# yu45020/Text_Segmentation_Image_Inpainting

Hardware: NVIDIA H100
Metric: PartialConv UNet 512x512 images/sec (fwd+bwd) (higher is better)
Workload: dtype bf16

## Files before the change

text_segmentation_image_inpainting_b200/csrc/conv_k2r.cu:

```cuda
#include <string.h>

#include <algorithm>

#include "pcb_common.cuh"

namespace {

constexpr int K2R_N = 32;
constexpr int K2R_CO = 3;
constexpr int K2R_TAPS = 9;

size_t rup256(size_t v) { return (v + 255) / 256 * 256; }
size_t zbytes(const pcb_conv *c) { return rup256(static_cast<size_t>(c->n) * (c->h >> 1) * (c->w >> 1) * K2R_N * sizeof(bf16)); }

}

K2rPlan pcb_k2r_plan(const pcb_conv *c) {
    K2rPlan K;
    memset(&K, 0, sizeof(K));
    if (!pcb_smallco_eligible(c)) return K;
    if (c->kh != 3 || c->kw != 3 || c->pad_h != 1 || c->pad_w != 1 || c->cout > K2R_CO || c->nparts != 2) return K;
    if (c->ho != c->h || c->wo != c->w || ((c->h | c->w) & 1)) return K;
    K.pu = c->parts[0].x_up ? 0 : 1;
    K.ps = 1 - K.pu;
    const pcb_part &u = c->parts[K.pu], &v = c->parts[K.ps];
    if (!u.x_up || v.x_up || u.c < 32 || (u.c & 7) || v.c > 4) return K;
    if ((u.mask && u.mask_up != 1) || (v.mask && v.mask_up != 0)) return K;
    K.cu = u.c; K.cs = v.c;
    K.choff_u = K.pu == 0 ? 0 : c->parts[0].c;
    K.choff_s = K.ps == 0 ? 0 : c->parts[0].c;
    pcb_conv &S = K.sub;
    S.n = c->n; S.h = c->h >> 1; S.w = c->w >> 1; S.cin = u.c; S.cout = K2R_N; S.kh = S.kw = 1; S.stride = 1; S.pad_h = S.pad_w = 0; S.dil = 1;
    S.groups = 1; S.ho = S.h; S.wo = S.w; S.dtype = PCB_BF16; S.nparts = 1;
    S.parts[0] = u; S.parts[0].x_up = 0; S.parts[0].mask_up = 0;
    if (!pcb_tc_eligible(&S)) return K;
    pcb_tc_weight_layout(&S, &K.sub_fe, &K.sub_de);
    K.sub_fe = (K.sub_fe + 63) / 64 * 64;
    K.sub_de = (K.sub_de + 63) / 64 * 64;
    K.fwd_extra = K.sub_fe + 2 * static_cast<size_t>(K2R_N) * K.cu;
    K.dg_extra = K.sub_de;
    K.workspace = zbytes(c) + rup256(sizeof(float) * K2R_N * K.cu) + pcb_tc_workspace(&S);
    K.ok = true;
    return K;
}

namespace {

__global__ void k2r_weight_kernel(const float *__restrict__ w, float *__restrict__ wsub, int cout, int cin, int choff_u, int cu) {
    const int i = blockIdx.x * blockDim.x + threadIdx.x;
    if (i >= K2R_N * cu) return;
    const int k = i / cu, ch = i - k * cu;
    const int tap = k / K2R_CO, co = k - tap * K2R_CO;
    wsub[i] = (tap < K2R_TAPS && co < cout) ? w[(static_cast<long long>(co) * K2R_TAPS + tap) * cin + choff_u + ch] : 0.f;
}

__global__ void k2r_dw_scatter_kernel(const float *__restrict__ dwsub, float *__restrict__ dw, int cout, int cin, int choff_u, int cu) {
    const int i = blockIdx.x * blockDim.x + threadIdx.x;
    if (i >= K2R_TAPS * K2R_CO * cu) return;
    const int k = i / cu, ch = i - k * cu;
    const int tap = k / K2R_CO, co = k - tap * K2R_CO;
    if (co < cout) dw[(static_cast<long long>(co) * K2R_TAPS + tap) * cin + choff_u + ch] += dwsub[i];
}

struct K2rParams {
    int n, h, w, hs, ws, cout, cin, no_guard;
    const bf16 *z;
    const bf16 *v; int v_cstride;
    const uint8_t *mv;
    const bf16 *w_fwd; long long kf; int ktap, koff_s;
    const float *bias, *msum;
    bf16 *y; int y_cstride;
    const bf16 *dc; int dc_cstride;
    bf16 *d;
    float *dw; int choff_s;
};

__device__ __forceinline__ void bf4_to_float(const uint2 r, float (&f)[4]) {
    const __nv_bfloat162 *h = reinterpret_cast<const __nv_bfloat162 *>(&r);
    const float2 a = __bfloat1622float2(h[0]), b = __bfloat1622float2(h[1]);
    f[0] = a.x; f[1] = a.y; f[2] = b.x; f[3] = b.y;
}

template <int CS>
__global__ void __launch_bounds__(256) k2r_combine_kernel(const K2rParams P) {
    __shared__ float4 s_w[K2R_TAPS * K2R_CO];
    for (int i = threadIdx.x; i < K2R_TAPS * K2R_CO; i += blockDim.x) {
        const int tap = i / K2R_CO, co = i - tap * K2R_CO;
        float wv[4] = {0.f, 0.f, 0.f, 0.f};
        if (co < P.cout)
            for (int ch = 0; ch < CS; ++ch) wv[ch] = __bfloat162float(P.w_fwd[static_cast<long long>(co) * P.kf + static_cast<long long>(tap) * P.ktap + P.koff_s + ch]);
        s_w[i] = make_float4(wv[0], wv[1], wv[2], wv[3]);
    }
    __syncthreads();
    const long long total = static_cast<long long>(P.n) * P.hs * P.ws;
    for (long long idx = blockIdx.x * static_cast<long long>(blockDim.x) + threadIdx.x; idx < total; idx += static_cast<long long>(gridDim.x) * blockDim.x) {
        const int sx = static_cast<int>(idx % P.ws);
        const long long t = idx / P.ws;
        const int sy = static_cast<int>(t % P.hs), img = static_cast<int>(t / P.hs);
        float acc[4][K2R_CO];
#pragma unroll
        for (int ch = 0; ch < 4; ++ch)
#pragma unroll
            for (int co = 0; co < K2R_CO; ++co) acc[ch][co] = 0.f;
#pragma unroll
        for (int dy = -1; dy <= 1; ++dy) {
            const int yy = sy + dy;
            if (yy < 0 || yy >= P.hs) continue;
#pragma unroll
            for (int dx = -1; dx <= 1; ++dx) {
                const int xx = sx + dx;
                if (xx < 0 || xx >= P.ws) continue;
                const uint4 *row = reinterpret_cast<const uint4 *>(P.z + ((static_cast<long long>(img) * P.hs + yy) * P.ws + xx) * K2R_N);
                float zf[K2R_N];
#pragma unroll
                for (int q = 0; q < 4; ++q) {
                    const uint4 r = __ldg(row + q);
                    const __nv_bfloat162 *h = reinterpret_cast<const __nv_bfloat162 *>(&r);
#pragma unroll
                    for (int e = 0; e < 4; ++e) {
                        const float2 f = __bfloat1622float2(h[e]);
                        zf[q * 8 + 2 * e] = f.x; zf[q * 8 + 2 * e + 1] = f.y;
                    }
                }
#pragma unroll
                for (int a = 0; a < 2; ++a)
#pragma unroll
                    for (int b = 0; b < 2; ++b)
#pragma unroll
                        for (int tr = 0; tr < 3; ++tr)
#pragma unroll
                            for (int tc = 0; tc < 3; ++tc) {
                                const int ny = (a + tr + 1) / 2 - 1, nx = (b + tc + 1) / 2 - 1;
                                if (ny == dy && nx == dx) {
#pragma unroll
                                    for (int co = 0; co < K2R_CO; ++co) acc[a * 2 + b][co] += zf[(tr * 3 + tc) * K2R_CO + co];
                                }
                            }
            }
        }
        float xv[4][4][CS];
#pragma unroll
        for (int i = 0; i < 4; ++i) {
            const int y = 2 * sy - 1 + i;
#pragma unroll
            for (int j = 0; j < 4; ++j) {
                const int x = 2 * sx - 1 + j;
                bool ok = y >= 0 && y < P.h && x >= 0 && x < P.w;
                const long long q = (static_cast<long long>(img) * P.h + (ok ? y : 0)) * P.w + (ok ? x : 0);
                if (ok && P.mv) ok = P.mv[q] != 0;
                float f[4] = {0.f, 0.f, 0.f, 0.f};
                if (ok) bf4_to_float(__ldg(reinterpret_cast<const uint2 *>(P.v + q * P.v_cstride)), f);
#pragma unroll
                for (int ch = 0; ch < CS; ++ch) xv[i][j][ch] = f[ch];
            }
        }
#pragma unroll
        for (int tr = 0; tr < 3; ++tr)
#pragma unroll
            for (int tc = 0; tc < 3; ++tc)
#pragma unroll
                for (int co = 0; co < K2R_CO; ++co) {
                    const float4 wv = s_w[(tr * 3 + tc) * K2R_CO + co];
                    const float wq[4] = {wv.x, wv.y, wv.z, wv.w};
#pragma unroll
                    for (int a = 0; a < 2; ++a)
#pragma unroll
                        for (int b = 0; b < 2; ++b)
#pragma unroll
                            for (int ch = 0; ch < CS; ++ch) acc[a * 2 + b][co] = fmaf(wq[ch], xv[a + tr][b + tc][ch], acc[a * 2 + b][co]);
                }
#pragma unroll
        for (int a = 0; a < 2; ++a)
#pragma unroll
            for (int b = 0; b < 2; ++b) {
                const long long q = (static_cast<long long>(img) * P.h + 2 * sy + a) * P.w + 2 * sx + b;
                const float s = P.msum ? P.msum[q] : 1.f;
                const bool hole = (s == 0.f) && !P.no_guard;
                const float inv = hole ? 0.f : 1.0f / s;
                float o[8] = {0.f, 0.f, 0.f, 0.f, 0.f, 0.f, 0.f, 0.f};
#pragma unroll
                for (int co = 0; co < K2R_CO; ++co)
                    if (co < P.cout && !hole) o[co] = acc[a * 2 + b][co] * inv + (P.bias ? P.bias[co] : 0.f);
                Vec8<bf16>::store(P.y + q * P.y_cstride, o);
            }
    }
}

template <bool WG, int CS>
__global__ void __launch_bounds__(256) k2r_dbuild_kernel(const K2rParams P) {
    __shared__ float s_dw[WG ? K2R_TAPS * K2R_CO * 4 : 1];
    if (WG) {
        for (int i = threadIdx.x; i < K2R_TAPS * K2R_CO * 4; i += blockDim.x) s_dw[i] = 0.f;
        __syncthreads();
    }
    float gw[WG ? K2R_TAPS * K2R_CO : 1][WG ? CS : 1];
    if (WG) {
#pragma unroll
        for (int k = 0; k < K2R_TAPS * K2R_CO; ++k)
#pragma unroll
            for (int ch = 0; ch < CS; ++ch) gw[k][ch] = 0.f;
    }
    const long long total = static_cast<long long>(P.n) * P.hs * P.ws;
    for (long long idx = blockIdx.x * static_cast<long long>(blockDim.x) + threadIdx.x; idx < total; idx += static_cast<long long>(gridDim.x) * blockDim.x) {
        const int sx = static_cast<int>(idx % P.ws);
        const long long t = idx / P.ws;
        const int sy = static_cast<int>(t % P.hs), img = static_cast<int>(t / P.hs);
        float win[4][4][K2R_CO];
#pragma unroll
        for (int i = 0; i < 4; ++i) {
            const int y = 2 * sy - 1 + i;
#pragma unroll
            for (int j = 0; j < 4; ++j) {
                const int x = 2 * sx - 1 + j;
                const bool ok = y >= 0 && y < P.h && x >= 0 && x < P.w;
                float f[4] = {0.f, 0.f, 0.f, 0.f};
                if (ok) bf4_to_float(__ldg(reinterpret_cast<const uint2 *>(P.dc + ((static_cast<long long>(img) * P.h + y) * P.w + x) * P.dc_cstride)), f);
#pragma unroll
                for (int co = 0; co < K2R_CO; ++co) win[i][j][co] = f[co];
            }
        }
        if (P.d) {
            float dv[K2R_N];
#pragma unroll
            for (int k = K2R_TAPS * K2R_CO; k < K2R_N; ++k) dv[k] = 0.f;
#pragma unroll
            for (int tr = 0; tr < 3; ++tr)
#pragma unroll
                for (int tc = 0; tc < 3; ++tc)
#pragma unroll
                    for (int co = 0; co < K2R_CO; ++co)
                        dv[(tr * 3 + tc) * K2R_CO + co] = (win[2 - tr][2 - tc][co] + win[2 - tr][3 - tc][co]) + (win[3 - tr][2 - tc][co] + win[3 - tr][3 - tc][co]);
            bf16 *row = P.d + idx * K2R_N;
#pragma unroll
            for (int q = 0; q < 4; ++q) {
                float o[8];
#pragma unroll
                for (int e = 0; e < 8; ++e) o[e] = dv[q * 8 + e];
                Vec8<bf16>::store(row + q * 8, o);
            }
        }
        if (WG) {
#pragma unroll
            for (int a = 0; a < 2; ++a)
#pragma unroll
                for (int b = 0; b < 2; ++b) {
                    const long long q = (static_cast<long long>(img) * P.h + 2 * sy + a) * P.w + 2 * sx + b;
                    float f[4] = {0.f, 0.f, 0.f, 0.f};
                    if (!P.mv || P.mv[q] != 0) bf4_to_float(__ldg(reinterpret_cast<const uint2 *>(P.v + q * P.v_cstride)), f);
#pragma unroll
                    for (int tr = 0; tr < 3; ++tr)
#pragma unroll
                        for (int tc = 0; tc < 3; ++tc)
#pragma unroll
                            for (int co = 0; co < K2R_CO; ++co)
#pragma unroll
                                for (int ch = 0; ch < CS; ++ch)
                                    gw[(tr * 3 + tc) * K2R_CO + co][ch] = fmaf(win[a - tr + 2][b - tc + 2][co], f[ch], gw[(tr * 3 + tc) * K2R_CO + co][ch]);
                }
        }
    }
    if (WG) {
        const int lane = threadIdx.x & 31;
#pragma unroll
        for (int k = 0; k < K2R_TAPS * K2R_CO; ++k)
#pragma unroll
            for (int ch = 0; ch < CS; ++ch) {
                const float v = warp_sum(gw[k][ch]);
                if (lane == 0) atomicAdd(&s_dw[k * 4 + ch], v);
            }
        __syncthreads();
        for (int i = threadIdx.x; i < K2R_TAPS * K2R_CO * 4; i += blockDim.x) {
            const int k = i >> 2, ch = i & 3;
            const int tap = k / K2R_CO, co = k - tap * K2R_CO;
            if (co < P.cout && ch < CS) atomicAdd(P.dw + (static_cast<long long>(co) * K2R_TAPS + tap) * P.cin + P.choff_s + ch, s_dw[i]);
        }
    }
}

void base(K2rParams &P, const pcb_conv *c, const K2rPlan &K) {
    memset(&P, 0, sizeof(P));
    P.n = c->n; P.h = c->h; P.w = c->w; P.hs = c->h >> 1; P.ws = c->w >> 1; P.cout = c->cout; P.cin = c->cin; P.no_guard = c->no_guard;
    const pcb_part &v = c->parts[K.ps];
    P.v = static_cast<const bf16 *>(v.x); P.v_cstride = v.x_cstride; P.mv = v.mask; P.choff_s = K.choff_s;
}

int grid_for(const pcb_conv *c, int per_sm) {
    const long long total = static_cast<long long>(c->n) * (c->h >> 1) * (c->w >> 1);
    return static_cast<int>(std::max<long long>(1, std::min<long long>((total + 255) / 256, static_cast<long long>(per_sm) * pcb_num_sms())));
}

bf16 *dgrad_scratch(size_t bytes) {
    static void *buf[PCB_MAX_DEVICES] = {};
    static size_t cap[PCB_MAX_DEVICES] = {};
    const int dev = pcb_cur_device();
    if (cap[dev] < bytes) {
        void *fresh = nullptr;
        if (cudaMalloc(&fresh, bytes) != cudaSuccess) { cudaGetLastError(); return nullptr; }
        buf[dev] = fresh;
        cap[dev] = bytes;
    }
    return static_cast<bf16 *>(buf[dev]);
}

}

int pcb_k2r_weight_prepare(const pcb_conv *c, const K2rPlan &K, const float *w_master, void *w_fwd_extra, void *w_dg_extra, bool zero_padding,
                           cudaStream_t st) {
    PCB_CHECK(K.ok && w_fwd_extra && w_dg_extra, "k2r weight prepare: not a kernel-to-row layer / missing operand buffers");
    float *wsub = reinterpret_cast<float *>(static_cast<bf16 *>(w_fwd_extra) + K.sub_fe);
    k2r_weight_kernel<<<(K2R_N * K.cu + 255) / 256, 256, 0, st>>>(w_master, wsub, c->cout, c->cin, K.choff_u, K.cu);
    PCB_LAUNCH_CHECK();
    return pcb_tc_weight_prepare(&K.sub, wsub, w_fwd_extra, w_dg_extra, zero_padding, st);
}

int pcb_k2r_forward(const pcb_conv *c, const K2rPlan &K, const pcb_smallco_layout &L, const void *w_fwd, const void *w_fwd_extra, const float *bias,
                    void *y, int y_cstride, const float *msum, void *workspace, cudaStream_t st) {
    PCB_CHECK(K.ok && workspace, "k2r forward: not a kernel-to-row layer / no workspace");
    PCB_CHECK(y_cstride % 8 == 0 && y_cstride >= 8 && (reinterpret_cast<uintptr_t>(y) & 15) == 0, "small-cout forward: y must be 16-byte aligned with a channel stride that is a multiple of 8");
    uint8_t *ws = static_cast<uint8_t *>(workspace);
    bf16 *z = reinterpret_cast<bf16 *>(ws);
    uint64_t *sub_ws = reinterpret_cast<uint64_t *>(ws + zbytes(c) + rup256(sizeof(float) * K2R_N * K.cu));
    if (int rc = pcb_tc_forward_ws(&K.sub, w_fwd_extra, nullptr, z, K2R_N, nullptr, sub_ws, false, nullptr, nullptr, st)) return rc;
    K2rParams P;
    base(P, c, K);
    P.z = z; P.w_fwd = static_cast<const bf16 *>(w_fwd); P.kf = L.kf; P.ktap = L.ktap; P.koff_s = L.koff[K.ps];
    P.bias = bias; P.msum = msum; P.y = static_cast<bf16 *>(y); P.y_cstride = y_cstride;
    if (K.cs <= 3) k2r_combine_kernel<3><<<grid_for(c, 8), 256, 0, st>>>(P);
    else k2r_combine_kernel<4><<<grid_for(c, 8), 256, 0, st>>>(P);
    PCB_LAUNCH_CHECK();
    return 0;
}

int pcb_k2r_dgrad(const pcb_conv *c, const K2rPlan &K, const pcb_smallco_layout &L, const void *dc, int dc_cstride, const void *w_dgrad,
                  const void *w_dg_extra, void *const *dx, const int *dx_cstride, cudaStream_t st) {
    PCB_CHECK(K.ok, "k2r dgrad: not a kernel-to-row layer");
    PCB_CHECK(dc_cstride % 8 == 0 && dc_cstride >= 8, "small-cout dgrad: dc channel stride must be a multiple of 8");
    if (dx[K.pu]) {
        bf16 *d = dgrad_scratch(zbytes(c));
        PCB_CHECK(d != nullptr, "k2r dgrad: scratch allocation failed");
        K2rParams P;
        base(P, c, K);
        P.dc = static_cast<const bf16 *>(dc); P.dc_cstride = dc_cstride; P.d = d;
        k2r_dbuild_kernel<false, 3><<<grid_for(c, 8), 256, 0, st>>>(P);
        PCB_LAUNCH_CHECK();
        void *dxs[1] = {dx[K.pu]};
        const int cs[1] = {dx_cstride[K.pu]};
        if (int rc = pcb_tc_dgrad(&K.sub, d, K2R_N, w_dg_extra, dxs, cs, st)) return rc;
    }
    if (dx[K.ps]) {
        void *dxl[2] = {nullptr, nullptr};
        dxl[K.ps] = dx[K.ps];
        return pcb_smallco_dgrad(c, L, dc, dc_cstride, w_dgrad, dxl, dx_cstride, st);
    }
    return 0;
}

int pcb_k2r_wgrad(const pcb_conv *c, const K2rPlan &K, const void *dc, int dc_cstride, float *dw, void *workspace, bool zero_dw, cudaStream_t st) {
    PCB_CHECK(K.ok && workspace, "k2r wgrad: not a kernel-to-row layer / no workspace");
    PCB_CHECK(dc_cstride % 8 == 0 && dc_cstride >= 8, "small-cout wgrad: dc channel stride must be a multiple of 8");
    if (zero_dw) PCB_CUDA(cudaMemsetAsync(dw, 0, sizeof(float) * c->cout * K2R_TAPS * c->cin, st));
    uint8_t *ws = static_cast<uint8_t *>(workspace);
    bf16 *d = reinterpret_cast<bf16 *>(ws);
    float *dwsub = reinterpret_cast<float *>(ws + zbytes(c));
    void *sub_ws = ws + zbytes(c) + rup256(sizeof(float) * K2R_N * K.cu);
    K2rParams P;
    base(P, c, K);
    P.dc = static_cast<const bf16 *>(dc); P.dc_cstride = dc_cstride; P.d = d; P.dw = dw;
    if (K.cs <= 3) k2r_dbuild_kernel<true, 3><<<grid_for(c, 3), 128, 0, st>>>(P);
    else k2r_dbuild_kernel<true, 4><<<grid_for(c, 2), 128, 0, st>>>(P);
    PCB_LAUNCH_CHECK();
    if (int rc = pcb_tc_wgrad(&K.sub, d, K2R_N, dwsub, sub_ws, true, st)) return rc;
    k2r_dw_scatter_kernel<<<(K2R_TAPS * K2R_CO * K.cu + 255) / 256, 256, 0, st>>>(dwsub, dw, c->cout, c->cin, K.choff_u, K.cu);
    PCB_LAUNCH_CHECK();
    return 0;
}
```

text_segmentation_image_inpainting_b200/csrc/conv_tc.cu:

```cuda
#include <cuda.h>
#include <stdlib.h>
#include <string.h>

#include <algorithm>

#include "pcb_common.cuh"
#include "pcb_ptx.cuh"

namespace {

constexpr int BLOCK_M = 128;
constexpr int BLOCK_K = 64;
constexpr int A_STAGE_BYTES = BLOCK_M * 128;
constexpr int NUM_PRODUCER_THREADS = 128;
constexpr int TC_MAX_PARTS = 2;
constexpr int MMA_WARPS = 8;
constexpr int MMA_THREADS = MMA_WARPS * 32;
constexpr int acc_pitch(int block_n) { return block_n + 4; }
constexpr int acc_stage_bytes(int block_n) { return BLOCK_M * acc_pitch(block_n) * 4; }

inline int rup(int v, int m) { return (v + m - 1) / m * m; }

struct TcPart {
    const bf16 *x;
// ... 2054 lines not shown
    return S;
}

struct SpWParams {
    int cout, taps, cin, kw, cout64, choff_u;
    int eoff[4], nex[4];
    int ybits[2][4], xbits[2][4];
    long long kd_sp;
};

__global__ void sp_weight_dg_kernel(const float *__restrict__ wm, const SpWParams W, bf16 *__restrict__ w_d) {
    const int ci = blockIdx.x;
    int slot = blockIdx.y, cls = 0;
    while (cls < 3 && slot >= W.eoff[cls + 1]) ++cls;
    slot -= W.eoff[cls];
    const int ey = slot / W.nex[cls], ex = slot - ey * W.nex[cls];
    const int yb = W.ybits[cls >> 1][ey], xb = W.xbits[cls & 1][ex];
    for (int co = threadIdx.x; co < W.cout; co += blockDim.x) {
        const float *wrow = wm + static_cast<long long>(co) * W.taps * W.cin + W.choff_u + ci;
        float v = 0.f;
        for (int tr = 0; tr < 4; ++tr)
            if ((yb >> tr) & 1)
                for (int tc = 0; tc < 4; ++tc)
                    if ((xb >> tc) & 1) v += wrow[static_cast<long long>(tr * W.kw + tc) * W.cin];
        w_d[static_cast<long long>(ci) * W.kd_sp + static_cast<long long>(W.eoff[cls] + slot) * W.cout64 + co] = __float2bfloat16_rn(v);
    }
}

int sp_weight_prepare(const pcb_conv *c, const SpPlan &S, const Layout &L, const float *w_master, bf16 *w_d, cudaStream_t st) {
    SpWParams W;
    memset(&W, 0, sizeof(W));
    W.cout = c->cout; W.taps = c->kh * c->kw; W.cin = c->cin; W.kw = c->kw; W.cout64 = L.cout64; W.kd_sp = S.kd_sp;
    for (int p = 0; p < S.pu; ++p) W.choff_u += c->parts[p].c;
    for (int cls = 0; cls < 4; ++cls) { W.eoff[cls] = S.eoff[cls]; W.nex[cls] = S.ax.ne[cls & 1]; }
    for (int q = 0; q < 2; ++q)
        for (int e = 0; e < 4; ++e) { W.ybits[q][e] = S.ay.tapbits[q][e]; W.xbits[q][e] = S.ax.tapbits[q][e]; }
    sp_weight_dg_kernel<<<dim3(c->parts[S.pu].c, S.net_total), 128, 0, st>>>(w_master, W, w_d);
    PCB_LAUNCH_CHECK();
    return 0;
}

template <int BLOCK_N>
int launch_sp_n(TcParams &P, const SpTable &TB, const CUtensorMap &tw, const CUtensorMap &ta, cudaStream_t st) {
    const size_t stage = A_STAGE_BYTES + static_cast<size_t>(BLOCK_N) * 128;
    const size_t fixed = tma_fixed_smem(BLOCK_N);
    P.stages = static_cast<int>(std::min<size_t>(MAX_RING, (MAX_SMEM - fixed) / stage));
    PCB_CHECK(P.stages >= 2, "sub-pixel conv: stage of %zu bytes does not fit twice", stage);
    const size_t smem = fixed + P.stages * stage;
    auto kern = pconv_tc_sp_kernel<BLOCK_N>;
    PCB_SMEM_OPT_IN(kern, MAX_SMEM);
    const int num_tiles = ((P.m_total + BLOCK_M - 1) / BLOCK_M) * (P.ncols / BLOCK_N);
    const int grid = std::min(num_tiles, pcb_num_sms());
    kern<<<grid, TMA_THREADS, smem, st>>>(P, TB, tw, ta);
    PCB_LAUNCH_CHECK();
    return 0;
}

int sp_dgrad_up(const pcb_conv *c, const SpPlan &S, const Layout &L, const void *dc, int dc_cstride, const bf16 *w_sp_dg, void *dx_u, int dx_cstride,
                int *flag, cudaStream_t st) {
    const int hs = c->h / 2, ws = c->w / 2;
    const long long m_src = static_cast<long long>(c->n) * hs * ws;
    TcParams P;
    base_params(P, c, L);
    P.h = hs; P.w = ws; P.m_total = static_cast<int>(m_src);
    P.sub = 1; P.py = 0; P.px = 0; P.fh = hs; P.fw = ws;
    P.nparts = 1;
    memset(P.parts, 0, sizeof(P.parts));
    TcPart &pt = P.parts[0];
    pt.c = c->parts[S.pu].c; pt.c8 = S.c8_u; pt.kext = S.kext_u; pt.koff = 0; pt.mask = c->parts[S.pu].mask; pt.mup = 0;
    pt.dx = static_cast<bf16 *>(dx_u); pt.dx_cstride = dx_cstride;
    PCB_CHECK(dx_cstride % 8 == 0 && dx_cstride >= S.c8_u && (reinterpret_cast<uintptr_t>(dx_u) & 15) == 0, "sub-pixel dgrad: dx must be 16-byte aligned with a channel stride that is a multiple of 8");
    P.dc = static_cast<const bf16 *>(dc); P.dc_cstride = dc_cstride; P.dc_c8 = rup(c->cout, 8); P.dc_kext = L.cout64;
    P.abort_flag = flag;
    P.ncols = S.kext_u;
    P.box_w = S.bw; P.box_h = S.bh; P.box_n = S.bn;
    const int bn = S.block_n;
    SpTable TB;
    memset(&TB, 0, sizeof(TB));
    int ni = 0;
    for (int cls = 0; cls < 4; ++cls) {
        const int py = cls >> 1, px = cls & 1;
        const int ney = S.ay.ne[py], nex = S.ax.ne[px];
        for (int e = 0; e < ney; ++e)
            for (int f = 0; f < nex; ++f) {
                SpItem &it = TB.it[ni++];
                it.dx = px - 2 * (S.ax.e0[px] + f); it.dy = py - 2 * (S.ay.e0[py] + e);
                it.wk = (S.eoff[cls] + e * nex + f) * L.cout64;
            }
    }
    TB.n_items = ni;
    CUtensorMap ta, tw;
    if (int rc = make_tmap_nhwc(&ta, dc, P.dc_c8, c->wo, c->ho, c->n, dc_cstride, S.bw, S.bh, S.bn, 2)) return rc;
    if (int rc = make_tmap_2d(&tw, w_sp_dg, rup(S.kext_u, 128), S.kd_sp, S.kd_sp, bn)) return rc;
    return (bn == 64) ? launch_sp_n<64>(P, TB, tw, ta, st) : launch_sp_n<32>(P, TB, tw, ta, st);
}

enum TcRoute { ROUTE_NONE, ROUTE_STEM, ROUTE_K2R, ROUTE_SMALLCO, ROUTE_TMA, ROUTE_TMA_S2, ROUTE_GATHER };

struct DirPlan {
    TcRoute route;
    int box_w, box_h, box_n;
    int bn;
    bool halo;
};

struct TcPlan {
    bool ok;
    Layout L;
    long long m_out, m_in;
    size_t fwd_elems, dg_elems;
    size_t extra_fwd_off, extra_dg_off;
    size_t sp_off;
    size_t workspace;
    size_t up_off[TC_MAX_PARTS];
    DirPlan fwd, dg, wg;
    bool fwd_tapmask, wg_tapmask;
    StemPlan stem;
    K2rPlan k2r;
    SpPlan sp;
    bool cls_halo[4];
    bool cls_fork;
    bool fuses_epilogue;
    bool dg_fuses_relu;
    bool dg_at_source;
};

TcPlan tc_plan(const pcb_conv *c) {
    TcPlan T;
    memset(&T, 0, sizeof(T));
    T.sp.pu = T.sp.ps = -1;
    if (!common_ok(c)) return T;
    T.ok = true;
    const int sms = pcb_num_sms();
    T.L = layout_of(c);
    const Layout &L = T.L;
    T.m_out = static_cast<long long>(c->n) * c->ho * c->wo;
    T.m_in = static_cast<long long>(c->n) * c->h * c->w;
    bool any_mask = false;
    for (int p = 0; p < c->nparts; ++p) any_mask = any_mask || (c->parts[p].mask != nullptr);
    const bool smallco = !L.rowpack && pcb_smallco_eligible(c);
    if (L.rowpack) T.stem = pcb_stem_plan(c);
    if (smallco) T.k2r = pcb_k2r_plan(c);
    const bool stem = T.stem.ok, k2r = T.k2r.ok;
    if (!L.rowpack && !smallco) T.sp = sp_plan(c, L, sms);

    T.fwd_elems = static_cast<size_t>(L.rows_f) * L.kf;
    T.sp_off = static_cast<size_t>(rup(L.ktap, 128)) * L.kd;
    T.dg_elems = L.rowpack ? 0 : T.sp_off;
    if (T.sp.ok) T.dg_elems += static_cast<size_t>(T.sp.sp_dg_elems);
    T.extra_fwd_off = (T.fwd_elems + 63) / 64 * 64;
    T.extra_dg_off = (T.sp_off + 63) / 64 * 64;
    if (k2r) {
        T.fwd_elems = T.extra_fwd_off + T.k2r.fwd_extra;
        T.dg_elems = T.extra_dg_off + T.k2r.dg_extra;
    }
    if (stem) T.fwd_elems = T.extra_fwd_off + T.stem.fwd_extra;

    int bw, bh, bn;
    const bool fwd_tma = tma_fwd_ok(c, &bw, &bh, &bn);
    DirPlan &F = T.fwd;
    if (stem) F.route = ROUTE_STEM;
    else if (k2r) F.route = ROUTE_K2R;
    else if (smallco) F.route = ROUTE_SMALLCO;
    else if (fwd_tma) {
        F.route = ROUTE_TMA;
        F.box_w = bw; F.box_h = bh; F.box_n = bn;
        F.bn = pick_bn(c->cout <= 32 ? 32 : L.rows_f, T.m_out, true, sms);
        F.halo = c->stride == 1 && c->kh <= 8 && halo_ok(c->kw, c->dil, bw, bh, bn, F.bn);
        T.fwd_tapmask = any_mask && !F.halo;
    } else {
        F.route = ROUTE_GATHER;
        F.bn = L.bn_f;
        T.fwd_tapmask = true;
    }

    DirPlan &D = T.dg;
    if (k2r) D.route = ROUTE_K2R;
    else if (smallco) D.route = ROUTE_SMALLCO;
    else if (L.rowpack) D.route = ROUTE_NONE;
    else if (c->stride == 1 && tile_box(c->w, c->h, &bw, &bh, &bn)) {
        D.route = ROUTE_TMA;
        D.box_w = bw; D.box_h = bh; D.box_n = bn;
        D.bn = pick_bn(L.ktap, T.m_in, false, sms);
        D.halo = c->kh <= 8 && halo_ok(c->kw, c->dil, bw, bh, bn, D.bn);
    } else if (tma_dgrad_s2_ok(c, &bw, &bh, &bn)) {
        D.route = ROUTE_TMA_S2;
        D.box_w = bw; D.box_h = bh; D.box_n = bn;
        const long long m_class = static_cast<long long>(c->n) * (c->h / 2) * (c->w / 2);
        D.bn = pick_bn(L.ktap, m_class, false, sms);
        for (int cls = 0; cls < 4; ++cls) T.cls_halo[cls] = halo_ok(class_kw(c, cls & 1), 1, bw, bh, bn, D.bn);
        T.cls_fork = ((m_class + BLOCK_M - 1) / BLOCK_M) * (L.ktap / D.bn) < sms;
    } else {
        D.route = ROUTE_GATHER;
        D.bn = (L.ktap % 128 == 0) ? 128 : 64;
    }

    const bool wg_tma = tma_wgrad_ok(c, &bw, &bh, &bn);
    DirPlan &W = T.wg;
    if (stem) W.route = ROUTE_STEM;
    else if (k2r) W.route = ROUTE_K2R;
    else if (smallco) W.route = ROUTE_SMALLCO;
    else if (wg_tma) {
        W.route = ROUTE_TMA;
        W.box_w = bw; W.box_h = bh; W.box_n = bn;
        W.halo = c->stride == 1 && c->kw == 3 && bw == 64 && bh == 1 && bn == 1 && 64 + (c->kw - 1) * c->dil <= 256;
        W.bn = (c->cout > 64 && T.m_out >= 128 * 64) ? 128 : 64;
        T.wg_tapmask = any_mask;
    } else {
        W.route = ROUTE_GATHER;
        T.wg_tapmask = true;
    }

    if (k2r) T.workspace = T.k2r.workspace;
    else if (stem) T.workspace = std::max(T.stem.workspace, tapmask_bytes(c));
    else {
        T.workspace = tapmask_bytes(c);
        if (fwd_tma || wg_tma)
            for (int p = 0; p < c->nparts; ++p)
                if (c->parts[p].x_up) { T.up_off[p] = T.workspace; T.workspace += up_bytes(c, p); }
    }

    T.fuses_epilogue = !smallco;
    T.dg_fuses_relu = c->nparts == 1 && !T.sp.ok && D.route == ROUTE_TMA;
    T.dg_at_source = smallco ? k2r : T.sp.ok;
    return T;
}

int a_operand_maps(const pcb_conv *c, const TcPlan &T, void *workspace, int bx, int by, int bn, CUtensorMap (&ta)[TC_MAX_PARTS],
                   int *use_fix, cudaStream_t st) {
    memset(ta, 0, sizeof(ta));
    for (int p = 0; p < c->nparts; ++p) {
        const pcb_part &pt = c->parts[p];
        const void *src = pt.x;
        long long cs = pt.x_cstride;
        const int c8 = rup(pt.c, 8);
        if (pt.x_up) {
            bf16 *up = reinterpret_cast<bf16 *>(static_cast<uint8_t *>(workspace) + T.up_off[p]);
            const long long pix = static_cast<long long>(c->n) * (c->h >> 1) * (c->w >> 1);
            const long long work = pix * (c8 >> 3);
            const int grid = static_cast<int>(std::min<long long>((work + 255) / 256, 16ll * pcb_num_sms()));
            upsample_part_kernel<<<grid, 256, 0, st>>>(static_cast<const bf16 *>(pt.x), pt.x_cstride, c8, pix, c->h >> 1, c->w >> 1, up);
            PCB_LAUNCH_CHECK();
            src = up; cs = c8;
        }
        if (pt.mask) *use_fix = 1;
        if (int rc = make_tmap_nhwc(&ta[p], src, c8, c->w, c->h, c->n, cs, bx, by, bn, c->stride)) return rc;
    }
    if (c->nparts < 2) ta[1] = ta[0];
    return 0;
}

pcb_smallco_layout smallco_layout(const Layout &L) {
    pcb_smallco_layout S;
    S.ktap = L.ktap; S.koff[0] = L.koff[0]; S.koff[1] = L.koff[1]; S.cout64 = L.cout64; S.kf = L.kf; S.kd = L.kd;
    return S;
}

}

bool pcb_tc_eligible(const pcb_conv *c) { return common_ok(c); }

size_t pcb_tc_workspace(const pcb_conv *c) { return tc_plan(c).workspace; }

void pcb_tc_weight_layout(const pcb_conv *c, size_t *fwd_elems, size_t *dgrad_elems) {
    const TcPlan T = tc_plan(c);
    *fwd_elems = T.fwd_elems;
    *dgrad_elems = T.dg_elems;
}

bool pcb_tc_subpixel(const pcb_conv *c) { return tc_plan(c).dg_at_source; }

void pcb_tc_routes(const pcb_conv *c, int32_t routes[3]) {
    static const int32_t code[] = {PCB_ROUTE_NONE, PCB_ROUTE_STEM, PCB_ROUTE_K2R, PCB_ROUTE_SMALLCO, PCB_ROUTE_TMA, PCB_ROUTE_TMA_S2,
                                   PCB_ROUTE_GATHER};
    const TcPlan T = tc_plan(c);
    routes[0] = code[T.fwd.route]; routes[1] = code[T.dg.route]; routes[2] = code[T.wg.route];
}

int pcb_tc_weight_prepare(const pcb_conv *c, const float *w_master, void *w_fwd, void *w_dgrad, bool zero_padding, cudaStream_t st) {
    const TcPlan T = tc_plan(c);
    const Layout &L = T.L;
    const size_t fe = T.fwd_elems, de = T.dg_elems;
    if (zero_padding) {
        PCB_CUDA(cudaMemsetAsync(w_fwd, 0, fe * 2, st));
        if (w_dgrad && de) PCB_CUDA(cudaMemsetAsync(w_dgrad, 0, de * 2, st));
    }
    WPrepParams W;
    memset(&W, 0, sizeof(W));
    W.cout = c->cout; W.taps = c->kh * c->kw; W.cin = c->cin; W.kw = c->kw; W.rowpack = L.rowpack; W.nparts = c->nparts;
    W.ktap = L.ktap; W.cout64 = L.cout64; W.kf = L.kf; W.kd = L.kd;
    int off = 0;
    for (int p = 0; p < c->nparts; ++p) { W.choff[p] = off; W.c[p] = c->parts[p].c; W.koff[p] = L.koff[p]; off += c->parts[p].c; }
    bf16 *wf = static_cast<bf16 *>(w_fwd), *wd = static_cast<bf16 *>(w_dgrad);
    if (!L.rowpack && W.taps <= 65535 && c->cout >= 32 && c->cin >= 32) {
        dim3 tg((c->cin + 31) / 32, (c->cout + 31) / 32, W.taps);
        tc_weight_prepare_tiled_kernel<<<tg, 256, 0, st>>>(w_master, W, wf, (w_dgrad && de) ? wd : nullptr);
    } else {
        const long long total = static_cast<long long>(c->cout) * W.taps * c->cin;
        const int grid = static_cast<int>(std::min<long long>((total + 1023) / 1024, 8ll * pcb_num_sms()));
        tc_weight_prepare_kernel<<<grid < 1 ? 1 : grid, 256, 0, st>>>(w_master, W, wf, (w_dgrad && de) ? wd : nullptr);
    }
    PCB_LAUNCH_CHECK();
    if (T.fwd.route == ROUTE_STEM) return pcb_stem_weight_prepare(c, T.stem, w_master, wf + T.extra_fwd_off, zero_padding, st);
    if (T.fwd.route == ROUTE_K2R) {
        PCB_CHECK(w_dgrad != nullptr, "kernel-to-row weights need the dgrad operand buffer");
        return pcb_k2r_weight_prepare(c, T.k2r, w_master, wf + T.extra_fwd_off, wd + T.extra_dg_off, zero_padding, st);
    }
    if (T.sp.ok) {
        PCB_CHECK(w_dgrad != nullptr, "sub-pixel weights need the dgrad operand buffer");
        return sp_weight_prepare(c, T.sp, L, w_master, wd + T.sp_off, st);
    }
    return 0;
}

int pcb_tc_forward_mask_pass(const pcb_conv *c, uint64_t *tapmask, cudaStream_t st) {
    const TcPlan T = tc_plan(c);
    PCB_CHECK(T.m_out < (1ll << 31), "problem too large");
    return T.fwd_tapmask ? launch_tapmask(c, tapmask, st) : 0;
}

bool pcb_tc_fuses_epilogue(const pcb_conv *c) { return tc_plan(c).fuses_epilogue; }

int pcb_tc_forward_ws(const pcb_conv *c, const void *w_fwd, const float *bias, void *y, int y_cstride, const float *msum,
                      uint64_t *tapmask, bool mask_pass_done, double *bn_sums, const pcb_ep *ep, cudaStream_t st) {
    int *flag = abort_flag_ptr();
    PCB_CHECK(flag != nullptr, "cudaMalloc(abort flag) failed");
    const TcPlan T = tc_plan(c);
    const Layout &L = T.L;
    const DirPlan &F = T.fwd;
    PCB_CHECK(T.m_out < (1ll << 31), "problem too large");
    PCB_CHECK(y_cstride % 8 == 0 && y_cstride >= c->cout, "tensor-core forward: y channel stride must be a multiple of 8 and >= cout");
    PCB_CHECK(bn_sums == nullptr || T.fuses_epilogue, "fused BatchNorm statistics requested from a kernel that does not produce them");
    PCB_CHECK(ep == nullptr || T.fuses_epilogue, "fused BatchNorm + activation requested from a kernel that does not apply it");
    if (!mask_pass_done && T.fwd_tapmask)
        if (int rc = launch_tapmask(c, tapmask, st)) return rc;
    const bf16 *wf = static_cast<const bf16 *>(w_fwd);
    if (F.route == ROUTE_STEM) return pcb_stem_forward(c, T.stem, wf + T.extra_fwd_off, bias, y, y_cstride, msum, tapmask, bn_sums, ep, st);
    if (F.route == ROUTE_K2R) return pcb_k2r_forward(c, T.k2r, smallco_layout(L), w_fwd, wf + T.extra_fwd_off, bias, y, y_cstride, msum, tapmask, st);
    if (F.route == ROUTE_SMALLCO) return pcb_smallco_forward(c, smallco_layout(L), w_fwd, bias, y, y_cstride, msum, st);
    TcParams P;
    base_params(P, c, L);
    P.m_total = static_cast<int>(T.m_out);
    fill_parts(c, L, P.parts, tapmask, T.m_out);
    P.bias = bias; P.msum = msum; P.y = static_cast<bf16 *>(y); P.y_cstride = y_cstride; P.abort_flag = flag;
    P.bn_sums = bn_sums; P.bn_c = c->cout;
    set_ep(P, ep);
    P.ncols = L.rows_f;
    CUtensorMap tm;
    if (int rc = make_tmap_2d(&tm, w_fwd, L.rows_f, L.kf, L.kf, F.bn)) return rc;
    if (F.route == ROUTE_TMA) {
        P.box_w = F.box_w; P.box_h = F.box_h; P.box_n = F.box_n;
        CUtensorMap ta[TC_MAX_PARTS];
        if (int rc = a_operand_maps(c, T, tapmask, F.box_w + (F.halo ? (c->kw - 1) * c->dil : 0), F.box_h, F.box_n, ta, &P.use_fix, st)) return rc;
        P.ncols = (c->cout <= 32) ? 32 : L.rows_f;
        P.wk_base = 0; P.wk_col = L.ktap; P.wk_row = c->kw * L.ktap;
        return launch_tma<0>(P, tm, ta[0], ta[1], F.bn, F.halo, st);
    }
    return launch_tc<0>(P, tm, F.bn, st);
}

bool pcb_tc_dgrad_fuses_relu(const pcb_conv *c) { return tc_plan(c).dg_fuses_relu; }

int pcb_tc_dgrad(const pcb_conv *c, const void *dc, int dc_cstride, const void *w_dgrad, void *const *dx, const int *dx_cstride,
                 cudaStream_t st, const void *relu_x, int relu_cstride) {
    const TcPlan T = tc_plan(c);
    const Layout &L = T.L;
    const DirPlan &D = T.dg;
    PCB_CHECK(D.route != ROUTE_NONE, "data gradient of a row-packed (cin <= 8) tensor-core layer: set force_generic and pass KRSC weights");
    PCB_CHECK(w_dgrad != nullptr && (reinterpret_cast<uintptr_t>(dc) & 15) == 0, "pcb_pconv_backward_data: w_dgrad required / dc misaligned");
    PCB_CHECK(relu_x == nullptr || (T.dg_fuses_relu && relu_cstride % 8 == 0 && relu_cstride >= rup(c->cin, 8) &&
                                    (reinterpret_cast<uintptr_t>(relu_x) & 15) == 0),
              "tensor-core dgrad: the ReLU backward is fused only on the TMA-fed stride-1 kernel (16-byte aligned input, channel stride %% 8 == 0)");
    int *flag = abort_flag_ptr();
    PCB_CHECK(flag != nullptr, "cudaMalloc(abort flag) failed");
    PCB_CHECK(T.m_in < (1ll << 31), "problem too large");
    PCB_CHECK(dc_cstride % 8 == 0 && dc_cstride >= rup(c->cout, 8), "tensor-core dgrad: dc channel stride must be a multiple of 8");
    const bf16 *wd = static_cast<const bf16 *>(w_dgrad);
    if (D.route == ROUTE_K2R) return pcb_k2r_dgrad(c, T.k2r, smallco_layout(L), dc, dc_cstride, w_dgrad, wd + T.extra_dg_off, dx, dx_cstride, st);
    if (D.route == ROUTE_SMALLCO) return pcb_smallco_dgrad(c, smallco_layout(L), dc, dc_cstride, w_dgrad, dx, dx_cstride, st);
    const SpPlan &SPL = T.sp;
    void *dx_local[TC_MAX_PARTS] = {nullptr, nullptr};
    for (int p = 0; p < c->nparts && p < TC_MAX_PARTS; ++p) dx_local[p] = dx[p];
    if (SPL.ok) {
        if (dx[SPL.pu] != nullptr)
            if (int rc = sp_dgrad_up(c, SPL, L, dc, dc_cstride, wd + T.sp_off, dx[SPL.pu], dx_cstride[SPL.pu], flag, st)) return rc;
        dx_local[SPL.pu] = nullptr;
        if (SPL.ps < 0 || dx[SPL.ps] == nullptr) return 0;
    }
    dx = dx_local;
    TcParams P;
    base_params(P, c, L);
    P.m_total = static_cast<int>(T.m_in);
    fill_parts(c, L, P.parts, nullptr, 0);
    for (int p = 0; p < c->nparts; ++p) {
        P.parts[p].dx = static_cast<bf16 *>(dx[p]);
        P.parts[p].dx_cstride = dx_cstride[p];
        PCB_CHECK(!dx[p] || (dx_cstride[p] % 8 == 0 && dx_cstride[p] >= P.parts[p].c8 && (reinterpret_cast<uintptr_t>(dx[p]) & 15) == 0),
                  "tensor-core dgrad: dx[%d] must be 16-byte aligned with a channel stride that is a multiple of 8", p);
    }
    P.dc = static_cast<const bf16 *>(dc); P.dc_cstride = dc_cstride; P.dc_c8 = rup(c->cout, 8); P.dc_kext = L.cout64;
    P.relu_x = static_cast<const bf16 *>(relu_x); P.relu_cstride = relu_cstride;
    P.abort_flag = flag;
    P.ncols = L.ktap;
    CUtensorMap tm;
    if (int rc = make_tmap_2d(&tm, w_dgrad, rup(L.ktap, 128), L.kd, L.kd, D.bn)) return rc;
    if (D.route == ROUTE_TMA) {
        P.box_w = D.box_w; P.box_h = D.box_h; P.box_n = D.box_n;
        P.wk_base = 0; P.wk_col = L.cout64; P.wk_row = c->kw * L.cout64;
        CUtensorMap ta;
        if (int rc = make_tmap_nhwc(&ta, dc, P.dc_c8, c->wo, c->ho, c->n, dc_cstride, D.box_w + (D.halo ? (c->kw - 1) * c->dil : 0), D.box_h, D.box_n, 1)) return rc;
        return launch_tma<1>(P, tm, ta, ta, D.bn, D.halo, st);
    }
    if (D.route == ROUTE_TMA_S2) {
        const int hh = c->h / 2, hw = c->w / 2;
        P.box_w = D.box_w; P.box_h = D.box_h; P.box_n = D.box_n;
        const bool fork = T.cls_fork;
        ClassStreams *CS = nullptr;
        if (fork) {
            if (int rc = class_streams(&CS)) return rc;
            PCB_CUDA(cudaEventRecord(CS->ev_fork, st));
        }
        for (int cls = 0; cls < 4; ++cls) {
            TcParams Q = P;
            const int py = cls >> 1, px = cls & 1;
            const int tr0 = (py + c->pad_h) & 1, tc0 = (px + c->pad_w) & 1;
            Q.kh = (c->kh - tr0 + 1) / 2; Q.kw = class_kw(c, px);
            Q.pad_h = (py + c->pad_h - tr0) / 2; Q.pad_w = (px + c->pad_w - tc0) / 2;
            Q.h = hh; Q.w = hw; Q.stride = 1; Q.dil = 1;
            Q.m_total = static_cast<int>(static_cast<long long>(c->n) * hh * hw);
            Q.sub = 2; Q.py = py; Q.px = px; Q.fh = c->h; Q.fw = c->w;
            Q.wk_base = (tr0 * c->kw + tc0) * L.cout64; Q.wk_row = 2 * c->kw * L.cout64; Q.wk_col = 2 * L.cout64;
            const bool halo = T.cls_halo[cls];
            CUtensorMap ta;
            if (int rc = make_tmap_nhwc(&ta, dc, P.dc_c8, c->wo, c->ho, c->n, dc_cstride, Q.box_w + (halo ? Q.kw - 1 : 0), Q.box_h, Q.box_n, 1)) return rc;
            cudaStream_t cs = (fork && cls > 0) ? CS->aux[cls - 1] : st;
            if (fork && cls > 0) PCB_CUDA(cudaStreamWaitEvent(cs, CS->ev_fork, 0));
            if (int rc = launch_tma<1>(Q, tm, ta, ta, D.bn, halo, cs)) return rc;
            if (fork && cls > 0) {
                PCB_CUDA(cudaEventRecord(CS->ev_join[cls - 1], cs));
                PCB_CUDA(cudaStreamWaitEvent(st, CS->ev_join[cls - 1], 0));
            }
        }
        return 0;
    }
    return launch_tc<1>(P, tm, D.bn, st);
}


template <int BLOCK_N, int T, bool HALO>
int launch_wgrad_tma(WgParams &P, const CUtensorMap &tdc, const CUtensorMap &ta0, const CUtensorMap &ta1, cudaStream_t st) {
    const int rows_a = 64 + (HALO ? (P.kw - 1) * P.dil : 0);
    PCB_CHECK(rows_a <= (HALO ? 3 : 1) * WGRAD_FIX_THREADS, "TMA-fed wgrad: %d-row A blocks exceed the fixer warps", rows_a);
    const size_t a_blk = (static_cast<size_t>(rows_a) * 128 + 1023) / 1024 * 1024;
    const size_t stage = (HALO ? 1 : T) * 2 * a_blk + static_cast<size_t>(BLOCK_N) * 128;
    P.stages = static_cast<int>(std::min<size_t>(MAX_RING, RING_BUDGET / stage));
    PCB_CHECK(P.stages >= 2, "TMA-fed wgrad: stage of %zu bytes does not fit twice", stage);
    const size_t smem = 1024 + P.stages * stage + 24 * MAX_RING;
    auto kern = pconv_tc_wgrad_tma_kernel<BLOCK_N, T, HALO>;
    PCB_SMEM_OPT_IN(kern, MAX_SMEM);
    P.tap_groups = HALO ? P.kh : (P.kh * P.kw + T - 1) / T;
    P.ci_tiles = (P.ktap + 127) / 128;
    const int co_tiles = (P.cout + BLOCK_N - 1) / BLOCK_N;
    const int base_ctas = co_tiles * P.tap_groups * P.ci_tiles;
    const int total_kb = (P.m_total + 63) / 64;
    int splits = (2 * pcb_num_sms() + base_ctas - 1) / base_ctas;
    splits = std::max(1, std::min(splits, total_kb));
    splits = std::min(splits, 65535);
    P.kb_per_split = (total_kb + splits - 1) / splits;
    splits = (total_kb + P.kb_per_split - 1) / P.kb_per_split;
    dim3 grid(base_ctas, splits);
    kern<<<grid, WGRAD_TMA_THREADS, smem, st>>>(P, tdc, ta0, ta1);
    PCB_LAUNCH_CHECK();
    return 0;
}

template <int BLOCK_N, int T, int STAGES>
static int launch_wgrad(WgParams &P, const CUtensorMap &tm, int cout, cudaStream_t st) {
    constexpr size_t smem = 1024 + STAGES * (T * 16384 + BLOCK_N * 128) + 24 * STAGES;
    auto kern = pconv_tc_wgrad_kernel<BLOCK_N, T, STAGES>;
    PCB_SMEM_OPT_IN(kern, (int)smem);
    P.tap_groups = (P.ntaps + T - 1) / T;
    P.ci_tiles = (P.ktap + 127) / 128;
    const int co_tiles = (cout + BLOCK_N - 1) / BLOCK_N;
    const int base_ctas = co_tiles * P.tap_groups * P.ci_tiles;
    const int total_kb = (P.m_total + 63) / 64;
    int splits = (4 * pcb_num_sms() + base_ctas - 1) / base_ctas;
    splits = std::max(1, std::min(splits, total_kb));
    splits = std::min(splits, 65535);
    P.kb_per_split = (total_kb + splits - 1) / splits;
    splits = (total_kb + P.kb_per_split - 1) / P.kb_per_split;
    dim3 grid(base_ctas, splits);
    kern<<<grid, WGRAD_THREADS, smem, st>>>(P, tm);
    PCB_LAUNCH_CHECK();
    return 0;
}

int pcb_tc_wgrad(const pcb_conv *c, const void *dc, int dc_cstride, float *dw, void *workspace, bool zero_dw, cudaStream_t st) {
    int *flag = abort_flag_ptr();
    PCB_CHECK(flag != nullptr, "cudaMalloc(abort flag) failed");
    PCB_CHECK(workspace != nullptr, "pcb_tc_wgrad: workspace required");
    const TcPlan T = tc_plan(c);
    const Layout &L = T.L;
    const DirPlan &W = T.wg;
    PCB_CHECK(T.m_out < (1ll << 31), "problem too large");
    PCB_CHECK(dc_cstride % 8 == 0 && dc_cstride >= c->cout, "tensor-core wgrad: dc channel stride must be a multiple of 8");
    if (W.route == ROUTE_STEM) return pcb_stem_wgrad(c, T.stem, dc, dc_cstride, dw, workspace, zero_dw, st);
    if (W.route == ROUTE_K2R) return pcb_k2r_wgrad(c, T.k2r, dc, dc_cstride, dw, workspace, zero_dw, st);
    if (W.route == ROUTE_SMALLCO) return pcb_smallco_wgrad(c, smallco_layout(L), dc, dc_cstride, dw, zero_dw, st);
    uint64_t *tapmask = static_cast<uint64_t *>(workspace);
    if (T.wg_tapmask)
        if (int rc = launch_tapmask(c, tapmask, st)) return rc;
    const size_t dw_bytes = sizeof(float) * c->cout * c->kh * c->kw * c->cin;
    if (zero_dw) PCB_CUDA(cudaMemsetAsync(dw, 0, dw_bytes, st));
    WgParams P;
    memset(&P, 0, sizeof(P));
    P.n = c->n; P.h = c->h; P.w = c->w; P.cin = c->cin; P.cout = c->cout; P.kh = c->kh; P.kw = c->kw; P.stride = c->stride;
    P.pad_h = c->pad_h; P.pad_w = c->pad_w; P.dil = c->dil; P.ho = c->ho; P.wo = c->wo; P.m_total = static_cast<int>(T.m_out);
    P.nparts = c->nparts; P.rowpack = L.rowpack; P.ktap = L.ktap; P.ntaps = L.rowpack ? c->kh : c->kh * c->kw;
    fill_parts(c, L, P.parts, tapmask, T.m_out);
    P.dw = dw; P.abort_flag = flag;
    CUtensorMap tm;
    if (int rc = make_tmap_2d(&tm, dc, T.m_out, c->cout, dc_cstride, 64)) return rc;
    if (W.route == ROUTE_TMA) {
        P.box_w = W.box_w; P.box_h = W.box_h; P.box_n = W.box_n;
        CUtensorMap ta[TC_MAX_PARTS];
        if (int rc = a_operand_maps(c, T, workspace, W.box_w + (W.halo ? (c->kw - 1) * c->dil : 0), W.box_h, W.box_n, ta, &P.use_fix, st)) return rc;
        if (W.bn == 128) return W.halo ? launch_wgrad_tma<128, 3, true>(P, tm, ta[0], ta[1], st) : launch_wgrad_tma<128, 3, false>(P, tm, ta[0], ta[1], st);
        return W.halo ? launch_wgrad_tma<64, 3, true>(P, tm, ta[0], ta[1], st) : launch_wgrad_tma<64, 3, false>(P, tm, ta[0], ta[1], st);
    }
    return launch_wgrad<64, 3, 3>(P, tm, c->cout, st);
}

int pcb_tc_read_abort_flag(int *value) {
    int *flag = abort_flag_ptr();
    PCB_CHECK(flag != nullptr, "no abort flag");
    PCB_CUDA(cudaMemcpy(value, flag, sizeof(int), cudaMemcpyDeviceToHost));
    if (*value != 0) cudaMemset(flag, 0, sizeof(int));
    return 0;
}
```

text_segmentation_image_inpainting_b200/csrc/pcb_common.cuh:

```cuda
#pragma once
#include <cuda_bf16.h>
#include <cuda_runtime.h>
#include <stdint.h>
#include <stdio.h>

#include "../../include/pconv_b200.h"

int pcb_set_error(const char *fmt, ...);
void pcb_count_launch(int n = 1);

#define PCB_CHECK(cond, ...)                       \
    do {                                           \
        if (!(cond)) return pcb_set_error(__VA_ARGS__); \
    } while (0)

#define PCB_CUDA(expr)                                                                           \
    do {                                                                                         \
        cudaError_t _e = (expr);                                                                 \
        if (_e != cudaSuccess)                                                                   \
            return pcb_set_error("%s:%d: %s -> %s", __FILE__, __LINE__, #expr, cudaGetErrorString(_e)); \
    } while (0)

#define PCB_LAUNCH_CHECK()                                                                        \
    do {                                                                                         \
        cudaError_t _e = cudaGetLastError();                                                     \
        if (_e != cudaSuccess)                                                                   \
            return pcb_set_error("%s:%d: kernel launch -> %s", __FILE__, __LINE__, cudaGetErrorString(_e)); \
        pcb_count_launch();                                                                      \
    } while (0)

constexpr int PCB_MAX_DEVICES = 64;

static inline int pcb_cur_device() {
    int dev = 0;
    cudaGetDevice(&dev);
    return (dev >= 0 && dev < PCB_MAX_DEVICES) ? dev : 0;
}

static inline int pcb_num_sms() {
    static int sms[PCB_MAX_DEVICES] = {0};
    const int dev = pcb_cur_device();
    if (!sms[dev]) {
        int v = 0;
        cudaDeviceGetAttribute(&v, cudaDevAttrMultiProcessorCount, dev);
        sms[dev] = v > 0 ? v : 132;
    }
    return sms[dev];
}

#define PCB_SMEM_OPT_IN(kern, bytes)                                                                          \
    do {                                                                                                      \
        static bool pcb_done_[PCB_MAX_DEVICES] = {};                                                          \
        const int pcb_dev_ = pcb_cur_device();                                                                \
        if (!pcb_done_[pcb_dev_]) {                                                                           \
            PCB_CUDA(cudaFuncSetAttribute(kern, cudaFuncAttributeMaxDynamicSharedMemorySize, (int)(bytes))); \
            pcb_done_[pcb_dev_] = true;                                                                       \
        }                                                                                                     \
    } while (0)

static inline size_t pcb_dtype_size(int dtype) { return dtype == PCB_BF16 ? 2 : 4; }

typedef __nv_bfloat16 bf16;

template <typename T> __device__ __forceinline__ float to_f32(T v);
template <> __device__ __forceinline__ float to_f32<float>(float v) { return v; }
template <> __device__ __forceinline__ float to_f32<bf16>(bf16 v) { return __bfloat162float(v); }

template <typename T> __device__ __forceinline__ T from_f32(float v);
template <> __device__ __forceinline__ float from_f32<float>(float v) { return v; }
template <> __device__ __forceinline__ bf16 from_f32<bf16>(float v) { return __float2bfloat16_rn(v); }

__device__ __forceinline__ float apply_act(float z, int act, float slope) {
    if (act == PCB_ACT_RELU) return z > 0.f ? z : 0.f;
    if (act == PCB_ACT_LEAKY) return z > 0.f ? z : z * slope;
    if (act == PCB_ACT_RELU6) return fminf(fmaxf(z, 0.f), 6.f);
    return z;
}
__device__ __forceinline__ float act_grad(float z, int act, float slope) {
    if (act == PCB_ACT_RELU) return z > 0.f ? 1.f : 0.f;
    if (act == PCB_ACT_LEAKY) return z > 0.f ? 1.f : slope;
    if (act == PCB_ACT_RELU6) return (z > 0.f && z < 6.f) ? 1.f : 0.f;
    return 1.f;
}

template <typename T> struct Vec8;
template <> struct Vec8<bf16> {
    static __device__ __forceinline__ void load(const bf16 *p, float (&v)[8]) {
        uint4 r = *reinterpret_cast<const uint4 *>(p);
        const __nv_bfloat162 *h = reinterpret_cast<const __nv_bfloat162 *>(&r);
#pragma unroll
        for (int i = 0; i < 4; ++i) {
            float2 f = __bfloat1622float2(h[i]);
            v[2 * i] = f.x;
            v[2 * i + 1] = f.y;
        }
    }
    static __device__ __forceinline__ void store(bf16 *p, const float (&v)[8]) {
        uint4 r;
        __nv_bfloat162 *h = reinterpret_cast<__nv_bfloat162 *>(&r);
#pragma unroll
        for (int i = 0; i < 4; ++i) h[i] = __floats2bfloat162_rn(v[2 * i], v[2 * i + 1]);
        *reinterpret_cast<uint4 *>(p) = r;
    }
};
template <> struct Vec8<float> {
    static __device__ __forceinline__ void load(const float *p, float (&v)[8]) {
        float4 a = reinterpret_cast<const float4 *>(p)[0], b = reinterpret_cast<const float4 *>(p)[1];
        v[0] = a.x; v[1] = a.y; v[2] = a.z; v[3] = a.w; v[4] = b.x; v[5] = b.y; v[6] = b.z; v[7] = b.w;
    }
    static __device__ __forceinline__ void store(float *p, const float (&v)[8]) {
        reinterpret_cast<float4 *>(p)[0] = make_float4(v[0], v[1], v[2], v[3]);
        reinterpret_cast<float4 *>(p)[1] = make_float4(v[4], v[5], v[6], v[7]);
    }
};

__device__ __forceinline__ float warp_sum(float v) {
#pragma unroll
    for (int o = 16; o > 0; o >>= 1) v += __shfl_xor_sync(0xffffffffu, v, o);
    return v;
}

struct pcb_ep { const float *scale, *shift; int act; float slope; };

int pcb_generic_forward(const pcb_conv *c, const void *w, const float *bias, void *y, int y_cstride, const float *msum, cudaStream_t st);
int pcb_generic_dgrad(const pcb_conv *c, const void *dc, int dc_cstride, const void *w_krsc, void *const *dx, const int *dx_cstride,
                      cudaStream_t st);
int pcb_generic_wgrad(const pcb_conv *c, const void *dc, int dc_cstride, float *dw, bool zero_dw, cudaStream_t st);
int pcb_mask_sums(const pcb_conv *c, float *msum, uint8_t *newmask, cudaStream_t st);
bool pcb_tc_eligible(const pcb_conv *c);
size_t pcb_tc_workspace(const pcb_conv *c);
void pcb_tc_weight_layout(const pcb_conv *c, size_t *fwd_elems, size_t *dgrad_elems);
int pcb_tc_weight_prepare(const pcb_conv *c, const float *w_master, void *w_fwd, void *w_dgrad, bool zero_padding, cudaStream_t st);
int pcb_tc_forward_mask_pass(const pcb_conv *c, uint64_t *tapmask, cudaStream_t st);
int pcb_tc_forward_ws(const pcb_conv *c, const void *w_fwd, const float *bias, void *y, int y_cstride, const float *msum,
                      uint64_t *tapmask, bool mask_pass_done, double *bn_sums, const pcb_ep *ep, cudaStream_t st);
bool pcb_tc_fuses_epilogue(const pcb_conv *c);
bool pcb_tc_subpixel(const pcb_conv *c);
int pcb_tc_dgrad(const pcb_conv *c, const void *dc, int dc_cstride, const void *w_dgrad, void *const *dx, const int *dx_cstride,
                 cudaStream_t st, const void *relu_x = nullptr, int relu_cstride = 0);
bool pcb_tc_dgrad_fuses_relu(const pcb_conv *c);
int pcb_tc_wgrad(const pcb_conv *c, const void *dc, int dc_cstride, float *dw, void *workspace, bool zero_dw, cudaStream_t st);
int pcb_tc_read_abort_flag(int *value);
void pcb_tc_routes(const pcb_conv *c, int32_t routes[3]);
struct pcb_smallco_layout { int ktap, koff[2], cout64; long long kf, kd; };
bool pcb_smallco_eligible(const pcb_conv *c);
int pcb_smallco_forward(const pcb_conv *c, const pcb_smallco_layout &L, const void *w_fwd, const float *bias, void *y, int y_cstride, const float *msum,
                        cudaStream_t st);
int pcb_smallco_dgrad(const pcb_conv *c, const pcb_smallco_layout &L, const void *dc, int dc_cstride, const void *w_dgrad, void *const *dx, const int *dx_cstride,
                      cudaStream_t st);
int pcb_smallco_wgrad(const pcb_conv *c, const pcb_smallco_layout &L, const void *dc, int dc_cstride, float *dw, bool zero_dw, cudaStream_t st);
struct K2rPlan {
    bool ok;
    int pu, ps;
    int cu, cs, choff_u, choff_s;
    pcb_conv sub;
    size_t sub_fe, sub_de;
    size_t fwd_extra, dg_extra;
    size_t workspace;
};
K2rPlan pcb_k2r_plan(const pcb_conv *c);
int pcb_k2r_weight_prepare(const pcb_conv *c, const K2rPlan &K, const float *w_master, void *w_fwd_extra, void *w_dg_extra, bool zero_padding,
                           cudaStream_t st);
int pcb_k2r_forward(const pcb_conv *c, const K2rPlan &K, const pcb_smallco_layout &L, const void *w_fwd, const void *w_fwd_extra, const float *bias,
                    void *y, int y_cstride, const float *msum, void *workspace, cudaStream_t st);
int pcb_k2r_dgrad(const pcb_conv *c, const K2rPlan &K, const pcb_smallco_layout &L, const void *dc, int dc_cstride, const void *w_dgrad,
                  const void *w_dg_extra, void *const *dx, const int *dx_cstride, cudaStream_t st);
int pcb_k2r_wgrad(const pcb_conv *c, const K2rPlan &K, const void *dc, int dc_cstride, float *dw, void *workspace, bool zero_dw, cudaStream_t st);
struct StemPlan {
    bool ok;
    pcb_conv sub;
    size_t sub_fe;
    size_t fwd_extra;
    size_t workspace;
};
StemPlan pcb_stem_plan(const pcb_conv *c);
int pcb_stem_weight_prepare(const pcb_conv *c, const StemPlan &K, const float *w_master, void *w_fwd_extra, bool zero_padding, cudaStream_t st);
int pcb_stem_forward(const pcb_conv *c, const StemPlan &K, const void *w_fwd_extra, const float *bias, void *y, int y_cstride,
                     const float *msum, void *workspace, double *bn_sums, const pcb_ep *ep, cudaStream_t st);
int pcb_stem_wgrad(const pcb_conv *c, const StemPlan &K, const void *dc, int dc_cstride, float *dw, void *workspace, bool zero_dw,
                   cudaStream_t st);
bool pcb_dw_eligible(const pcb_conv *c);
int pcb_dw_weight_prepare(const pcb_conv *c, const float *w_master, void *w_t, cudaStream_t st);
int pcb_dw_forward(const pcb_conv *c, const void *w_t, const float *bias, void *y, int y_cstride, const float *msum, double *bn_sums,
                   const pcb_ep *ep, cudaStream_t st);
int pcb_dw_dgrad(const pcb_conv *c, const void *dc, int dc_cstride, const void *w_t, void *dx, int dx_cstride, cudaStream_t st);
int pcb_dw_wgrad(const pcb_conv *c, const void *dc, int dc_cstride, float *dw, bool zero_dw, cudaStream_t st);
```

Baseline: 1125.

## Fuse kernel-to-row GEMM into tiled combine/dbuild kernels with in-kernel mma

The separate 1x1 tensor-core GEMM that produced the Z intermediate, and the dgrad/wgrad GEMMs over the D scratch, are folded into tiled kernels. These load upsampled-input halos via cp.async into shared memory and run mma.sync there, keeping the intermediate on-chip. The weight-prepare step is removed, and launches use persistent resident grids sized from occupancy. This removes global round trips for the 32-channel intermediate and several launches, at the cost of more shared memory, a channel cap of 72, and more complex kernels.

```diff
diff --git a/text_segmentation_image_inpainting_b200/csrc/conv_k2r.cu b/text_segmentation_image_inpainting_b200/csrc/conv_k2r.cu
--- a/text_segmentation_image_inpainting_b200/csrc/conv_k2r.cu
+++ b/text_segmentation_image_inpainting_b200/csrc/conv_k2r.cu
@@ -9,6 +9,18 @@
 constexpr int K2R_N = 32;
 constexpr int K2R_CO = 3;
 constexpr int K2R_TAPS = 9;
+constexpr int K2R_K = K2R_TAPS * K2R_CO;
+constexpr int K2R_MAX_CU = 72;
+
+constexpr int TY = 8, TX = 16, TPIX = TY * TX;
+constexpr int HY = TY + 2, HX = TX + 2, HPIX = HY * HX;
+constexpr int HROWS = (HPIX + 15) / 16 * 16;
+constexpr int OY = 2 * TY, OX = 2 * TX, OPIX = OY * OX;
+constexpr int CY = OY + 2, CX = OX + 2, CPIX = CY * CX;
+constexpr int THREADS = 128;
+constexpr int ZS = K2R_N + 1;
+constexpr int DS = K2R_N + 8;
+constexpr int DTS = TPIX + 8;
 
 size_t rup256(size_t v) { return (v + 255) / 256 * 256; }
 size_t zbytes(const pcb_conv *c) { return rup256(static_cast<size_t>(c->n) * (c->h >> 1) * (c->w >> 1) * K2R_N * sizeof(bf16)); }
@@ -46,17 +58,9 @@
 
 namespace {
 
-__global__ void k2r_weight_kernel(const float *__restrict__ w, float *__restrict__ wsub, int cout, int cin, int choff_u, int cu) {
-    const int i = blockIdx.x * blockDim.x + threadIdx.x;
-    if (i >= K2R_N * cu) return;
-    const int k = i / cu, ch = i - k * cu;
-    const int tap = k / K2R_CO, co = k - tap * K2R_CO;
-    wsub[i] = (tap < K2R_TAPS && co < cout) ? w[(static_cast<long long>(co) * K2R_TAPS + tap) * cin + choff_u + ch] : 0.f;
-}
-
 __global__ void k2r_dw_scatter_kernel(const float *__restrict__ dwsub, float *__restrict__ dw, int cout, int cin, int choff_u, int cu) {
     const int i = blockIdx.x * blockDim.x + threadIdx.x;
-    if (i >= K2R_TAPS * K2R_CO * cu) return;
+    if (i >= K2R_K * cu) return;
     const int k = i / cu, ch = i - k * cu;
     const int tap = k / K2R_CO, co = k - tap * K2R_CO;
     if (co < cout) dw[(static_cast<long long>(co) * K2R_TAPS + tap) * cin + choff_u + ch] += dwsub[i];
@@ -64,15 +68,18 @@
 
 struct K2rParams {
     int n, h, w, hs, ws, cout, cin, no_guard;
-    const bf16 *z;
+    int tiles_x, tiles_y, num_tiles;
+    const bf16 *u; int u_cstride, cu, ks, ups;
+    const uint8_t *mu;
     const bf16 *v; int v_cstride;
     const uint8_t *mv;
-    const bf16 *w_fwd; long long kf; int ktap, koff_s;
+    const bf16 *w_fwd; long long kf; int ktap, koff_u, koff_s;
+    const bf16 *w_dg; long long kd; int cout64;
     const float *bias, *msum;
     bf16 *y; int y_cstride;
     const bf16 *dc; int dc_cstride;
-    bf16 *d;
-    float *dw; int choff_s;
+    bf16 *du; int du_cstride;
+    float *dw, *dwsub; int choff_s;
 };
 
 __device__ __forceinline__ void bf4_to_float(const uint2 r, float (&f)[4]) {
@@ -81,271 +88,509 @@
     f[0] = a.x; f[1] = a.y; f[2] = b.x; f[3] = b.y;
 }
 
+__device__ __forceinline__ uint32_t smem_addr(const void *p) { return static_cast<uint32_t>(__cvta_generic_to_shared(p)); }
+__device__ __forceinline__ void ldsm_x4(uint32_t addr, uint32_t (&r)[4]) {
+    asm volatile("ldmatrix.sync.aligned.m8n8.x4.shared.b16 {%0, %1, %2, %3}, [%4];" : "=r"(r[0]), "=r"(r[1]), "=r"(r[2]), "=r"(r[3]) : "r"(addr));
+}
+__device__ __forceinline__ void ldsm_x2(uint32_t addr, uint32_t (&r)[2]) {
+    asm volatile("ldmatrix.sync.aligned.m8n8.x2.shared.b16 {%0, %1}, [%2];" : "=r"(r[0]), "=r"(r[1]) : "r"(addr));
+}
+__device__ __forceinline__ void ldsm_x4_t(uint32_t addr, uint32_t (&r)[4]) {
+    asm volatile("ldmatrix.sync.aligned.m8n8.x4.trans.shared.b16 {%0, %1, %2, %3}, [%4];" : "=r"(r[0]), "=r"(r[1]), "=r"(r[2]), "=r"(r[3]) : "r"(addr));
+}
+__device__ __forceinline__ void ldsm_x2_t(uint32_t addr, uint32_t (&r)[2]) {
+    asm volatile("ldmatrix.sync.aligned.m8n8.x2.trans.shared.b16 {%0, %1}, [%2];" : "=r"(r[0]), "=r"(r[1]) : "r"(addr));
+}
+__device__ __forceinline__ void mma_16816(float (&d)[4], const uint32_t (&a)[4], uint32_t b0, uint32_t b1) {
+    asm volatile("mma.sync.aligned.m16n8k16.row.col.f32.bf16.bf16.f32 {%0, %1, %2, %3}, {%4, %5, %6, %7}, {%8, %9}, {%0, %1, %2, %3};"
+                 : "+f"(d[0]), "+f"(d[1]), "+f"(d[2]), "+f"(d[3])
+                 : "r"(a[0]), "r"(a[1]), "r"(a[2]), "r"(a[3]), "r"(b0), "r"(b1));
+}
+__device__ __forceinline__ void cp_async16(uint32_t dst, const void *src, bool valid) {
+    const uint32_t sz = valid ? 16u : 0u;
+    asm volatile("cp.async.cg.shared.global [%0], [%1], 16, %2;" ::"r"(dst), "l"(src), "r"(sz) : "memory");
+}
+__device__ __forceinline__ void cp_async_wait_all() { asm volatile("cp.async.wait_all;" ::: "memory"); }
+
+__device__ __forceinline__ void tile_origin(const K2rParams &P, int tile, int &img, int &sy0, int &sx0) {
+    const int per_img = P.tiles_x * P.tiles_y;
+    img = tile / per_img;
+    const int r = tile - img * per_img;
+    const int ty = r / P.tiles_x;
+    sy0 = ty * TY;
+    sx0 = (r - ty * P.tiles_x) * TX;
+}
+
+__device__ __forceinline__ void load_u_tile(const K2rParams &P, uint8_t *su, uint8_t *sv, int img, int sy0, int sx0, int cols, int npix, int nch) {
+#pragma unroll
+    for (int r = 0; r < 2; ++r) {
+        const int pix = threadIdx.x + r * THREADS;
+        if (pix < npix) {
+            const int ty = pix / cols;
+            const int yy = sy0 + ty, xx = sx0 + pix - ty * cols;
+            const bool in = yy >= 0 && yy < P.hs && xx >= 0 && xx < P.ws;
+            sv[pix] = in && (!P.mu || P.mu[(static_cast<long long>(img) * P.hs + yy) * P.ws + xx] != 0);
+        }
+    }
+    __syncthreads();
+    for (int i = threadIdx.x; i < npix * nch; i += THREADS) {
+        const int pix = i / nch, j = i - pix * nch;
+        const int ty = pix / cols;
+        const bool ok = sv[pix] && j * 8 < P.cu;
+        const long long q = ok ? (static_cast<long long>(img) * P.hs + sy0 + ty) * P.ws + sx0 + pix - ty * cols : 0;
+        cp_async16(smem_addr(su + pix * P.ups + j * 16), P.u + (ok ? q * P.u_cstride + j * 8 : 0), ok);
+    }
+}
+
+__device__ __forceinline__ void load_dc_window(const K2rParams &P, int img, int sy, int sx, float (&win)[4][4][K2R_CO]) {
+#pragma unroll
+    for (int i = 0; i < 4; ++i) {
+        const int y = 2 * sy - 1 + i;
+#pragma unroll
+        for (int j = 0; j < 4; ++j) {
+            const int x = 2 * sx - 1 + j;
+            const bool ok = y >= 0 && y < P.h && x >= 0 && x < P.w;
+            float f[4] = {0.f, 0.f, 0.f, 0.f};
+            if (ok) bf4_to_float(__ldg(reinterpret_cast<const uint2 *>(P.dc + ((static_cast<long long>(img) * P.h + y) * P.w + x) * P.dc_cstride)), f);
+#pragma unroll
+            for (int co = 0; co < K2R_CO; ++co) win[i][j][co] = f[co];
+        }
+    }
+}
+
+__device__ __forceinline__ float d_entry(const float (&win)[4][4][K2R_CO], int tr, int tc, int co) {
+    return (win[2 - tr][2 - tc][co] + win[2 - tr][3 - tc][co]) + (win[3 - tr][2 - tc][co] + win[3 - tr][3 - tc][co]);
+}
+
 template <int CS>
-__global__ void __launch_bounds__(256) k2r_combine_kernel(const K2rParams P) {
-    __shared__ float4 s_w[K2R_TAPS * K2R_CO];
-    for (int i = threadIdx.x; i < K2R_TAPS * K2R_CO; i += blockDim.x) {
+__device__ __forceinline__ void k2r_combine_pixel(const K2rParams &P, const float *sz, const float4 *s_w, int img, int sy, int sx, int ly, int lx) {
+    float acc2[4][K2R_CO];
+#pragma unroll
+    for (int ch = 0; ch < 4; ++ch)
+#pragma unroll
+        for (int co = 0; co < K2R_CO; ++co) acc2[ch][co] = 0.f;
+#pragma unroll
+    for (int dy = -1; dy <= 1; ++dy)
+#pragma unroll
+        for (int dx = -1; dx <= 1; ++dx) {
+            const float *zr = sz + ((ly + 1 + dy) * HX + lx + 1 + dx) * ZS;
+#pragma unroll
+            for (int a = 0; a < 2; ++a)
+#pragma unroll
+                for (int b = 0; b < 2; ++b)
+#pragma unroll
+                    for (int tr = 0; tr < 3; ++tr)
+#pragma unroll
+                        for (int tc = 0; tc < 3; ++tc) {
+                            const int ny = (a + tr + 1) / 2 - 1, nx = (b + tc + 1) / 2 - 1;
+                            if (ny == dy && nx == dx) {
+#pragma unroll
+                                for (int co = 0; co < K2R_CO; ++co) acc2[a * 2 + b][co] += zr[(tr * 3 + tc) * K2R_CO + co];
+                            }
+                        }
+        }
+    float xv[4][4][CS];
+#pragma unroll
+    for (int i = 0; i < 4; ++i) {
+        const int y = 2 * sy - 1 + i;
+#pragma unroll
+        for (int j = 0; j < 4; ++j) {
+            const int x = 2 * sx - 1 + j;
+            const bool in = y >= 0 && y < P.h && x >= 0 && x < P.w;
+            const long long q = (static_cast<long long>(img) * P.h + (in ? y : 0)) * P.w + (in ? x : 0);
+            float f[4] = {0.f, 0.f, 0.f, 0.f};
+            if (in) bf4_to_float(__ldg(reinterpret_cast<const uint2 *>(P.v + q * P.v_cstride)), f);
+            const bool ok = in && (!P.mv || P.mv[q] != 0);
+#pragma unroll
+            for (int ch = 0; ch < CS; ++ch) xv[i][j][ch] = ok ? f[ch] : 0.f;
+        }
+    }
+#pragma unroll
+    for (int tr = 0; tr < 3; ++tr)
+#pragma unroll
+        for (int tc = 0; tc < 3; ++tc)
+#pragma unroll
+            for (int co = 0; co < K2R_CO; ++co) {
+                const float4 wv = s_w[(tr * 3 + tc) * K2R_CO + co];
+                const float wq[4] = {wv.x, wv.y, wv.z, wv.w};
+#pragma unroll
+                for (int a = 0; a < 2; ++a)
+#pragma unroll
+                    for (int b = 0; b < 2; ++b)
+#pragma unroll
+                        for (int ch = 0; ch < CS; ++ch) acc2[a * 2 + b][co] = fmaf(wq[ch], xv[a + tr][b + tc][ch], acc2[a * 2 + b][co]);
+            }
+#pragma unroll
+    for (int a = 0; a < 2; ++a)
+#pragma unroll
+        for (int b = 0; b < 2; ++b) {
+            const long long q = (static_cast<long long>(img) * P.h + 2 * sy + a) * P.w + 2 * sx + b;
+            const float s = P.msum ? P.msum[q] : 1.f;
+            const bool hole = (s == 0.f) && !P.no_guard;
+            const float inv = hole ? 0.f : 1.0f / s;
+            float o[8] = {0.f, 0.f, 0.f, 0.f, 0.f, 0.f, 0.f, 0.f};
+#pragma unroll
+            for (int co = 0; co < K2R_CO; ++co)
+                if (co < P.cout && !hole) o[co] = acc2[a * 2 + b][co] * inv + (P.bias ? P.bias[co] : 0.f);
+            Vec8<bf16>::store(P.y + q * P.y_cstride, o);
+        }
+}
+
+template <int CS>
+__global__ void __launch_bounds__(THREADS) k2r_combine_kernel(const K2rParams P) {
+    extern __shared__ __align__(16) uint8_t smem[];
+    __shared__ float4 s_w[K2R_K];
+    uint8_t *su = smem;
+    uint8_t *sw = smem + max(HROWS * P.ups, HPIX * ZS * 4);
+    float *sz = reinterpret_cast<float *>(smem);
+    const int tid = threadIdx.x, warp = tid >> 5, lane = tid & 31, g = lane >> 2, t = lane & 3;
+    __shared__ uint8_t s_valid[HPIX];
+    const int kc = P.ks * 16;
+    for (int i = tid; i < K2R_N * kc; i += THREADS) {
+        const int k = i / kc, ch = i - k * kc;
+        const int tap = k / K2R_CO, co = k - tap * K2R_CO;
+        reinterpret_cast<bf16 *>(sw + k * P.ups)[ch] =
+            (k < K2R_K && co < P.cout && ch < P.cu) ? P.w_fwd[static_cast<long long>(co) * P.kf + static_cast<long long>(tap) * P.ktap + P.koff_u + ch]
+                                                    : __float2bfloat16(0.f);
+    }
+    for (int i = tid; i < K2R_K; i += THREADS) {
         const int tap = i / K2R_CO, co = i - tap * K2R_CO;
         float wv[4] = {0.f, 0.f, 0.f, 0.f};
         if (co < P.cout)
             for (int ch = 0; ch < CS; ++ch) wv[ch] = __bfloat162float(P.w_fwd[static_cast<long long>(co) * P.kf + static_cast<long long>(tap) * P.ktap + P.koff_s + ch]);
         s_w[i] = make_float4(wv[0], wv[1], wv[2], wv[3]);
     }
-    __syncthreads();
-    const long long total = static_cast<long long>(P.n) * P.hs * P.ws;
-    for (long long idx = blockIdx.x * static_cast<long long>(blockDim.x) + threadIdx.x; idx < total; idx += static_cast<long long>(gridDim.x) * blockDim.x) {
-        const int sx = static_cast<int>(idx % P.ws);
-        const long long t = idx / P.ws;
-        const int sy = static_cast<int>(t % P.hs), img = static_cast<int>(t / P.hs);
-        float acc[4][K2R_CO];
-#pragma unroll
-        for (int ch = 0; ch < 4; ++ch)
-#pragma unroll
-            for (int co = 0; co < K2R_CO; ++co) acc[ch][co] = 0.f;
-#pragma unroll
-        for (int dy = -1; dy <= 1; ++dy) {
-            const int yy = sy + dy;
-            if (yy < 0 || yy >= P.hs) continue;
-#pragma unroll
-            for (int dx = -1; dx <= 1; ++dx) {
-                const int xx = sx + dx;
-                if (xx < 0 || xx >= P.ws) continue;
-                const uint4 *row = reinterpret_cast<const uint4 *>(P.z + ((static_cast<long long>(img) * P.hs + yy) * P.ws + xx) * K2R_N);
-                float zf[K2R_N];
-#pragma unroll
-                for (int q = 0; q < 4; ++q) {
-                    const uint4 r = __ldg(row + q);
-                    const __nv_bfloat162 *h = reinterpret_cast<const __nv_bfloat162 *>(&r);
-#pragma unroll
-                    for (int e = 0; e < 4; ++e) {
-                        const float2 f = __bfloat1622float2(h[e]);
-                        zf[q * 8 + 2 * e] = f.x; zf[q * 8 + 2 * e + 1] = f.y;
+    const int ly = tid / TX, lx = tid - ly * TX;
+    for (int tile = blockIdx.x; tile < P.num_tiles; tile += gridDim.x) {
+        int img, sy0, sx0;
+        tile_origin(P, tile, img, sy0, sx0);
+        load_u_tile(P, su, s_valid, img, sy0 - 1, sx0 - 1, HX, HPIX, P.ks * 2);
+        cp_async_wait_all();
+        __syncthreads();
+        float acc[3][4][4];
+#pragma unroll
+        for (int mi = 0; mi < 3; ++mi)
+#pragma unroll
+            for (int nt = 0; nt < 4; ++nt)
+#pragma unroll
+                for (int e = 0; e < 4; ++e) acc[mi][nt][e] = 0.f;
+        for (int kstep = 0; kstep < P.ks; ++kstep) {
+            uint32_t b[4][2];
+#pragma unroll
+            for (int nt = 0; nt < 4; ++nt) ldsm_x2(smem_addr(sw + (nt * 8 + (lane & 7)) * P.ups + kstep * 32 + ((lane >> 3) & 1) * 16), b[nt]);
+#pragma unroll
+            for (int mi = 0; mi < 3; ++mi) {
+                uint32_t a[4];
+                ldsm_x4(smem_addr(su + ((warp + 4 * mi) * 16 + (lane & 7) + ((lane >> 3) & 1) * 8) * P.ups + kstep * 32 + (lane >> 4) * 16), a);
+#pragma unroll
+                for (int nt = 0; nt < 4; ++nt) mma_16816(acc[mi][nt], a, b[nt][0], b[nt][1]);
+            }
+        }
+        __syncthreads();
+#pragma unroll
+        for (int mi = 0; mi < 3; ++mi)
+#pragma unroll
+            for (int h = 0; h < 2; ++h) {
+                const int r = (warp + 4 * mi) * 16 + g + 8 * h;
+                if (r < HPIX)
+#pragma unroll
+                    for (int nt = 0; nt < 4; ++nt) {
+                        sz[r * ZS + nt * 8 + 2 * t] = acc[mi][nt][2 * h];
+                        sz[r * ZS + nt * 8 + 2 * t + 1] = acc[mi][nt][2 * h + 1];
                     }
-                }
-#pragma unroll
-                for (int a = 0; a < 2; ++a)
-#pragma unroll
-                    for (int b = 0; b < 2; ++b)
-#pragma unroll
-                        for (int tr = 0; tr < 3; ++tr)
-#pragma unroll
-                            for (int tc = 0; tc < 3; ++tc) {
-                                const int ny = (a + tr + 1) / 2 - 1, nx = (b + tc + 1) / 2 - 1;
-                                if (ny == dy && nx == dx) {
-#pragma unroll
-                                    for (int co = 0; co < K2R_CO; ++co) acc[a * 2 + b][co] += zf[(tr * 3 + tc) * K2R_CO + co];
-                                }
-                            }
-            }
-        }
-        float xv[4][4][CS];
-#pragma unroll
-        for (int i = 0; i < 4; ++i) {
-            const int y = 2 * sy - 1 + i;
-#pragma unroll
-            for (int j = 0; j < 4; ++j) {
-                const int x = 2 * sx - 1 + j;
-                bool ok = y >= 0 && y < P.h && x >= 0 && x < P.w;
-                const long long q = (static_cast<long long>(img) * P.h + (ok ? y : 0)) * P.w + (ok ? x : 0);
-                if (ok && P.mv) ok = P.mv[q] != 0;
-                float f[4] = {0.f, 0.f, 0.f, 0.f};
-                if (ok) bf4_to_float(__ldg(reinterpret_cast<const uint2 *>(P.v + q * P.v_cstride)), f);
-#pragma unroll
-                for (int ch = 0; ch < CS; ++ch) xv[i][j][ch] = f[ch];
-            }
-        }
-#pragma unroll
-        for (int tr = 0; tr < 3; ++tr)
-#pragma unroll
-            for (int tc = 0; tc < 3; ++tc)
-#pragma unroll
-                for (int co = 0; co < K2R_CO; ++co) {
-                    const float4 wv = s_w[(tr * 3 + tc) * K2R_CO + co];
-                    const float wq[4] = {wv.x, wv.y, wv.z, wv.w};
-#pragma unroll
-                    for (int a = 0; a < 2; ++a)
-#pragma unroll
-                        for (int b = 0; b < 2; ++b)
-#pragma unroll
-                            for (int ch = 0; ch < CS; ++ch) acc[a * 2 + b][co] = fmaf(wq[ch], xv[a + tr][b + tc][ch], acc[a * 2 + b][co]);
-                }
-#pragma unroll
-        for (int a = 0; a < 2; ++a)
-#pragma unroll
-            for (int b = 0; b < 2; ++b) {
-                const long long q = (static_cast<long long>(img) * P.h + 2 * sy + a) * P.w + 2 * sx + b;
-                const float s = P.msum ? P.msum[q] : 1.f;
-                const bool hole = (s == 0.f) && !P.no_guard;
-                const float inv = hole ? 0.f : 1.0f / s;
-                float o[8] = {0.f, 0.f, 0.f, 0.f, 0.f, 0.f, 0.f, 0.f};
-#pragma unroll
-                for (int co = 0; co < K2R_CO; ++co)
-                    if (co < P.cout && !hole) o[co] = acc[a * 2 + b][co] * inv + (P.bias ? P.bias[co] : 0.f);
-                Vec8<bf16>::store(P.y + q * P.y_cstride, o);
-            }
-    }
-}
-
-template <bool WG, int CS>
-__global__ void __launch_bounds__(256) k2r_dbuild_kernel(const K2rParams P) {
-    __shared__ float s_dw[WG ? K2R_TAPS * K2R_CO * 4 : 1];
-    if (WG) {
-        for (int i = threadIdx.x; i < K2R_TAPS * K2R_CO * 4; i += blockDim.x) s_dw[i] = 0.f;
-        __syncthreads();
-    }
-    float gw[WG ? K2R_TAPS * K2R_CO : 1][WG ? CS : 1];
-    if (WG) {
-#pragma unroll
-        for (int k = 0; k < K2R_TAPS * K2R_CO; ++k)
-#pragma unroll
-            for (int ch = 0; ch < CS; ++ch) gw[k][ch] = 0.f;
-    }
-    const long long total = static_cast<long long>(P.n) * P.hs * P.ws;
-    for (long long idx = blockIdx.x * static_cast<long long>(blockDim.x) + threadIdx.x; idx < total; idx += static_cast<long long>(gridDim.x) * blockDim.x) {
-        const int sx = static_cast<int>(idx % P.ws);
-        const long long t = idx / P.ws;
-        const int sy = static_cast<int>(t % P.hs), img = static_cast<int>(t / P.hs);
-        float win[4][4][K2R_CO];
-#pragma unroll
-        for (int i = 0; i < 4; ++i) {
-            const int y = 2 * sy - 1 + i;
-#pragma unroll
-            for (int j = 0; j < 4; ++j) {
-                const int x = 2 * sx - 1 + j;
-                const bool ok = y >= 0 && y < P.h && x >= 0 && x < P.w;
-                float f[4] = {0.f, 0.f, 0.f, 0.f};
-                if (ok) bf4_to_float(__ldg(reinterpret_cast<const uint2 *>(P.dc + ((static_cast<long long>(img) * P.h + y) * P.w + x) * P.dc_cstride)), f);
-#pragma unroll
-                for (int co = 0; co < K2R_CO; ++co) win[i][j][co] = f[co];
-            }
-        }
-        if (P.d) {
+            }
+        __syncthreads();
+        if (sy0 + ly < P.hs && sx0 + lx < P.ws) k2r_combine_pixel<CS>(P, sz, s_w, img, sy0 + ly, sx0 + lx, ly, lx);
+        __syncthreads();
+    }
+}
+
+__device__ __forceinline__ void k2r_dgrad_tiles(const K2rParams &P) {
+    constexpr int OS = K2R_MAX_CU + 8;
+    __shared__ __align__(16) bf16 sd[TPIX * DS];
+    __shared__ __align__(16) bf16 swt[K2R_MAX_CU * DS];
+    __shared__ __align__(16) bf16 so[TPIX * OS];
+    const int tid = threadIdx.x, warp = tid >> 5, lane = tid & 31, g = lane >> 2, t = lane & 3;
+    constexpr int WPT = K2R_MAX_CU * K2R_N / THREADS;
+#pragma unroll
+    for (int r = 0; r < WPT; ++r) {
+        const int i = tid + r * THREADS;
+        const int ch = i / K2R_N, k = i - ch * K2R_N;
+        const int tap = k / K2R_CO, co = k - tap * K2R_CO;
+        if (ch < P.cu)
+            swt[ch * DS + k] = (k < K2R_K && co < P.cout) ? P.w_dg[static_cast<long long>(P.koff_u + ch) * P.kd + tap * P.cout64 + co] : __float2bfloat16(0.f);
+    }
+    const int nch = P.cu / 8;
+    for (int tile = blockIdx.x; tile < P.num_tiles; tile += gridDim.x) {
+        int img, sy0, sx0;
+        tile_origin(P, tile, img, sy0, sx0);
+        {
+            const int ly = tid / TX, lx = tid - ly * TX;
+            const int sy = sy0 + ly, sx = sx0 + lx;
             float dv[K2R_N];
 #pragma unroll
-            for (int k = K2R_TAPS * K2R_CO; k < K2R_N; ++k) dv[k] = 0.f;
-#pragma unroll
-            for (int tr = 0; tr < 3; ++tr)
-#pragma unroll
-                for (int tc = 0; tc < 3; ++tc)
-#pragma unroll
-                    for (int co = 0; co < K2R_CO; ++co)
-                        dv[(tr * 3 + tc) * K2R_CO + co] = (win[2 - tr][2 - tc][co] + win[2 - tr][3 - tc][co]) + (win[3 - tr][2 - tc][co] + win[3 - tr][3 - tc][co]);
-            bf16 *row = P.d + idx * K2R_N;
+            for (int k = 0; k < K2R_N; ++k) dv[k] = 0.f;
+            if (sy < P.hs && sx < P.ws) {
+                float win[4][4][K2R_CO];
+                load_dc_window(P, img, sy, sx, win);
+#pragma unroll
+                for (int tr = 0; tr < 3; ++tr)
+#pragma unroll
+                    for (int tc = 0; tc < 3; ++tc)
+#pragma unroll
+                        for (int co = 0; co < K2R_CO; ++co) dv[(tr * 3 + tc) * K2R_CO + co] = d_entry(win, tr, tc, co);
+            }
 #pragma unroll
             for (int q = 0; q < 4; ++q) {
                 float o[8];
 #pragma unroll
                 for (int e = 0; e < 8; ++e) o[e] = dv[q * 8 + e];
-                Vec8<bf16>::store(row + q * 8, o);
-            }
-        }
-        if (WG) {
-#pragma unroll
-            for (int a = 0; a < 2; ++a)
-#pragma unroll
-                for (int b = 0; b < 2; ++b) {
-                    const long long q = (static_cast<long long>(img) * P.h + 2 * sy + a) * P.w + 2 * sx + b;
-                    float f[4] = {0.f, 0.f, 0.f, 0.f};
-                    if (!P.mv || P.mv[q] != 0) bf4_to_float(__ldg(reinterpret_cast<const uint2 *>(P.v + q * P.v_cstride)), f);
-#pragma unroll
-                    for (int tr = 0; tr < 3; ++tr)
-#pragma unroll
-                        for (int tc = 0; tc < 3; ++tc)
-#pragma unroll
-                            for (int co = 0; co < K2R_CO; ++co)
-#pragma unroll
-                                for (int ch = 0; ch < CS; ++ch)
-                                    gw[(tr * 3 + tc) * K2R_CO + co][ch] = fmaf(win[a - tr + 2][b - tc + 2][co], f[ch], gw[(tr * 3 + tc) * K2R_CO + co][ch]);
+                Vec8<bf16>::store(sd + tid * DS + q * 8, o);
+            }
+        }
+        __syncthreads();
+        uint32_t a[2][2][4];
+        float mrow[2][2];
+#pragma unroll
+        for (int mi = 0; mi < 2; ++mi) {
+            const int ly = warp * 2 + mi;
+#pragma unroll
+            for (int kstep = 0; kstep < 2; ++kstep)
+                ldsm_x4(smem_addr(sd + (ly * 16 + (lane & 7) + ((lane >> 3) & 1) * 8) * DS + kstep * 16 + (lane >> 4) * 8), a[mi][kstep]);
+#pragma unroll
+            for (int h = 0; h < 2; ++h) {
+                const int sy = sy0 + ly, sx = sx0 + g + 8 * h;
+                mrow[mi][h] = (sy < P.hs && sx < P.ws && (!P.mu || P.mu[(static_cast<long long>(img) * P.hs + sy) * P.ws + sx])) ? 1.f : 0.f;
+            }
+        }
+        for (int nt = 0; nt < nch; ++nt) {
+            uint32_t b[4];
+            ldsm_x4(smem_addr(swt + (nt * 8 + (lane & 7)) * DS + (lane >> 3) * 8), b);
+#pragma unroll
+            for (int mi = 0; mi < 2; ++mi) {
+                float d[4] = {0.f, 0.f, 0.f, 0.f};
+                mma_16816(d, a[mi][0], b[0], b[1]);
+                mma_16816(d, a[mi][1], b[2], b[3]);
+#pragma unroll
+                for (int h = 0; h < 2; ++h)
+                    *reinterpret_cast<__nv_bfloat162 *>(so + ((warp * 2 + mi) * 16 + g + 8 * h) * OS + nt * 8 + 2 * t) =
+                        __floats2bfloat162_rn(d[2 * h] * mrow[mi][h], d[2 * h + 1] * mrow[mi][h]);
+            }
+        }
+        __syncwarp();
+        for (int i = lane; i < 32 * nch; i += 32) {
+            const int r = i / nch, j = i - r * nch;
+            const int sy = sy0 + warp * 2 + (r >> 4), sx = sx0 + (r & 15);
+            if (sy < P.hs && sx < P.ws)
+                *reinterpret_cast<uint4 *>(P.du + ((static_cast<long long>(img) * P.hs + sy) * P.ws + sx) * P.du_cstride + j * 8) =
+                    *reinterpret_cast<const uint4 *>(so + ((warp * 2) * 16 + r) * OS + j * 8);
+        }
+        __syncthreads();
+    }
+}
+
+template <int CS>
+__device__ __forceinline__ void k2r_wgrad_tiles(const K2rParams &P) {
+    __shared__ __align__(16) bf16 sdt[K2R_N * DTS];
+    __shared__ __align__(16) uint8_t su[TPIX * ((K2R_MAX_CU / 8) | 1) * 16];
+    __shared__ __align__(16) uint8_t sdc[CPIX * 16];
+    __shared__ __align__(16) uint8_t svt[OPIX * 16];
+    __shared__ float s_dw[K2R_K * 4];
+    __shared__ uint8_t s_uok[TPIX], s_vok[OPIX];
+    const int tid = threadIdx.x, warp = tid >> 5, lane = tid & 31, g = lane >> 2, t = lane & 3;
+    for (int i = tid; i < K2R_K * 4; i += THREADS) s_dw[i] = 0.f;
+    for (int i = tid; i < (K2R_N - K2R_K) * TPIX; i += THREADS) sdt[(K2R_K + i / TPIX) * DTS + i % TPIX] = __float2bfloat16(0.f);
+    const int ntiles_n = P.cu / 8;
+    float acc[2][3][4], gacc[5][4];
+#pragma unroll
+    for (int mi = 0; mi < 2; ++mi)
+#pragma unroll
+        for (int j = 0; j < 3; ++j)
+#pragma unroll
+            for (int e = 0; e < 4; ++e) acc[mi][j][e] = 0.f;
+#pragma unroll
+    for (int mt = 0; mt < 5; ++mt)
+#pragma unroll
+        for (int e = 0; e < 4; ++e) gacc[mt][e] = 0.f;
+    const int ly = tid / TX, lx = tid - ly * TX;
+    for (int tile = blockIdx.x; tile < P.num_tiles; tile += gridDim.x) {
+        int img, sy0, sx0;
+        tile_origin(P, tile, img, sy0, sx0);
+        const int oy0 = 2 * sy0, ox0 = 2 * sx0;
+        {
+            const int sy = sy0 + ly, sx = sx0 + lx;
+            s_uok[tid] = sy < P.hs && sx < P.ws && (!P.mu || P.mu[(static_cast<long long>(img) * P.hs + sy) * P.ws + sx] != 0);
+        }
+#pragma unroll
+        for (int r = 0; r < OPIX / THREADS; ++r) {
+            const int pix = tid + r * THREADS, y = oy0 + (pix / OX), x = ox0 + (pix % OX);
+            s_vok[pix] = y < P.h && x < P.w && (!P.mv || P.mv[(static_cast<long long>(img) * P.h + y) * P.w + x] != 0);
+        }
+        __syncthreads();
+        for (int i = tid; i < TPIX * ntiles_n; i += THREADS) {
+            const int pix = i / ntiles_n, j = i - pix * ntiles_n;
+            const bool ok = s_uok[pix];
+            const long long q = (static_cast<long long>(img) * P.hs + sy0 + pix / TX) * P.ws + sx0 + pix % TX;
+            cp_async16(smem_addr(su + pix * P.ups + j * 16), P.u + (ok ? q * P.u_cstride + j * 8 : 0), ok);
+        }
+        for (int pix = tid; pix < OPIX; pix += THREADS) {
+            const bool ok = s_vok[pix];
+            const long long q = (static_cast<long long>(img) * P.h + oy0 + pix / OX) * P.w + ox0 + pix % OX;
+            cp_async16(smem_addr(svt + pix * 16), P.v + (ok ? q * P.v_cstride : 0), ok);
+        }
+        for (int pix = tid; pix < CPIX; pix += THREADS) {
+            const int y = oy0 - 1 + pix / CX, x = ox0 - 1 + pix % CX;
+            const bool ok = y >= 0 && y < P.h && x >= 0 && x < P.w;
+            const long long q = (static_cast<long long>(img) * P.h + y) * P.w + x;
+            cp_async16(smem_addr(sdc + pix * 16), P.dc + (ok ? q * P.dc_cstride : 0), ok);
+        }
+        cp_async_wait_all();
+        __syncthreads();
+        {
+            float win[4][4][K2R_CO];
+#pragma unroll
+            for (int i = 0; i < 4; ++i)
+#pragma unroll
+                for (int j = 0; j < 4; ++j) {
+                    float f[4];
+                    bf4_to_float(*reinterpret_cast<const uint2 *>(sdc + ((2 * ly + i) * CX + 2 * lx + j) * 16), f);
+#pragma unroll
+                    for (int co = 0; co < K2R_CO; ++co) win[i][j][co] = f[co];
                 }
-        }
-    }
-    if (WG) {
-        const int lane = threadIdx.x & 31;
-#pragma unroll
-        for (int k = 0; k < K2R_TAPS * K2R_CO; ++k)
-#pragma unroll
-            for (int ch = 0; ch < CS; ++ch) {
-                const float v = warp_sum(gw[k][ch]);
-                if (lane == 0) atomicAdd(&s_dw[k * 4 + ch], v);
-            }
-        __syncthreads();
-        for (int i = threadIdx.x; i < K2R_TAPS * K2R_CO * 4; i += blockDim.x) {
-            const int k = i >> 2, ch = i & 3;
-            const int tap = k / K2R_CO, co = k - tap * K2R_CO;
-            if (co < P.cout && ch < CS) atomicAdd(P.dw + (static_cast<long long>(co) * K2R_TAPS + tap) * P.cin + P.choff_s + ch, s_dw[i]);
-        }
-    }
+#pragma unroll
+            for (int tr = 0; tr < 3; ++tr)
+#pragma unroll
+                for (int tc = 0; tc < 3; ++tc)
+#pragma unroll
+                    for (int co = 0; co < K2R_CO; ++co)
+                        sdt[((tr * 3 + tc) * K2R_CO + co) * DTS + tid] = __float2bfloat16(d_entry(win, tr, tc, co));
+        }
+#pragma unroll 2
+        for (int kstep = 0; kstep < 8; ++kstep) {
+            const int py = warp * 4 + (kstep >> 1), px0 = (kstep & 1) * 16;
+            uint32_t b[2];
+            ldsm_x2_t(smem_addr(svt + (py * OX + px0 + (lane & 7) + ((lane >> 3) & 1) * 8) * 16), b);
+            const int jm = lane >> 3, px = px0 + (lane & 7) + 8 * (jm >> 1);
+#pragma unroll
+            for (int mt = 0; mt < 5; ++mt) {
+                const int tap = min(2 * mt + (jm & 1), K2R_TAPS - 1), tr = tap / 3, tc = tap - tr * 3;
+                uint32_t a[4];
+                ldsm_x4_t(smem_addr(sdc + ((py - tr + 2) * CX + px - tc + 2) * 16), a);
+                mma_16816(gacc[mt], a, b[0], b[1]);
+            }
+        }
+        __syncthreads();
+#pragma unroll 2
+        for (int kstep = 0; kstep < TPIX / 16; ++kstep) {
+            uint32_t a[2][4];
+#pragma unroll
+            for (int mi = 0; mi < 2; ++mi)
+                ldsm_x4(smem_addr(sdt + (mi * 16 + (lane & 7) + ((lane >> 3) & 1) * 8) * DTS + kstep * 16 + (lane >> 4) * 8), a[mi]);
+#pragma unroll
+            for (int j = 0; j < 3; ++j) {
+                const int nt = warp + 4 * j;
+                if (nt < ntiles_n) {
+                    uint32_t b[2];
+                    ldsm_x2_t(smem_addr(su + (kstep * 16 + (lane & 7) + ((lane >> 3) & 1) * 8) * P.ups + nt * 16), b);
+#pragma unroll
+                    for (int mi = 0; mi < 2; ++mi) mma_16816(acc[mi][j], a[mi], b[0], b[1]);
+                }
+            }
+        }
+        __syncthreads();
+    }
+#pragma unroll
+    for (int j = 0; j < 3; ++j) {
+        const int nt = warp + 4 * j;
+        if (nt >= ntiles_n) continue;
+#pragma unroll
+        for (int mi = 0; mi < 2; ++mi)
+#pragma unroll
+            for (int h = 0; h < 2; ++h) {
+                const int k = mi * 16 + g + 8 * h;
+                if (k < K2R_K) {
+                    atomicAdd(P.dwsub + k * P.cu + nt * 8 + 2 * t, acc[mi][j][2 * h]);
+                    atomicAdd(P.dwsub + k * P.cu + nt * 8 + 2 * t + 1, acc[mi][j][2 * h + 1]);
+                }
+            }
+    }
+#pragma unroll
+    for (int mt = 0; mt < 5; ++mt)
+#pragma unroll
+        for (int h = 0; h < 2; ++h)
+#pragma unroll
+            for (int e = 0; e < 2; ++e) {
+                const int tap = 2 * mt + h, ch = 2 * t + e;
+                if (tap < K2R_TAPS && g < K2R_CO && ch < CS) atomicAdd(&s_dw[(tap * K2R_CO + g) * 4 + ch], gacc[mt][2 * h + e]);
+            }
+    __syncthreads();
+    for (int i = tid; i < K2R_K * 4; i += THREADS) {
+        const int k = i >> 2, ch = i & 3;
+        const int tap = k / K2R_CO, co = k - tap * K2R_CO;
+        if (co < P.cout && ch < CS) atomicAdd(P.dw + (static_cast<long long>(co) * K2R_TAPS + tap) * P.cin + P.choff_s + ch, s_dw[i]);
+    }
+}
+
+template <bool WG, int CS>
+__global__ void __launch_bounds__(THREADS) k2r_dbuild_kernel(const K2rParams P) {
+    if constexpr (WG) k2r_wgrad_tiles<CS>(P);
+    else k2r_dgrad_tiles(P);
+}
+
+struct Resident { size_t smem; int per_sm; };
+int resident_grid(void (*kern)(const K2rParams), size_t smem, int tiles, Resident (&cache)[PCB_MAX_DEVICES]) {
+    Resident &r = cache[pcb_cur_device()];
+    if (!r.per_sm || r.smem != smem) {
+        int n = 0;
+        if (cudaOccupancyMaxActiveBlocksPerMultiprocessor(&n, kern, THREADS, smem) != cudaSuccess) { cudaGetLastError(); n = 1; }
+        r.smem = smem; r.per_sm = std::max(n, 1);
+    }
+    return std::max(1, std::min(tiles, r.per_sm * pcb_num_sms()));
 }
 
 void base(K2rParams &P, const pcb_conv *c, const K2rPlan &K) {
     memset(&P, 0, sizeof(P));
     P.n = c->n; P.h = c->h; P.w = c->w; P.hs = c->h >> 1; P.ws = c->w >> 1; P.cout = c->cout; P.cin = c->cin; P.no_guard = c->no_guard;
-    const pcb_part &v = c->parts[K.ps];
+    P.tiles_x = (P.ws + TX - 1) / TX; P.tiles_y = (P.hs + TY - 1) / TY; P.num_tiles = P.n * P.tiles_x * P.tiles_y;
+    const pcb_part &u = c->parts[K.pu], &v = c->parts[K.ps];
+    P.u = static_cast<const bf16 *>(u.x); P.u_cstride = u.x_cstride; P.mu = u.mask; P.cu = K.cu; P.ks = (K.cu + 15) / 16;
     P.v = static_cast<const bf16 *>(v.x); P.v_cstride = v.x_cstride; P.mv = v.mask; P.choff_s = K.choff_s;
 }
 
-int grid_for(const pcb_conv *c, int per_sm) {
-    const long long total = static_cast<long long>(c->n) * (c->h >> 1) * (c->w >> 1);
-    return static_cast<int>(std::max<long long>(1, std::min<long long>((total + 255) / 256, static_cast<long long>(per_sm) * pcb_num_sms())));
-}
-
-bf16 *dgrad_scratch(size_t bytes) {
-    static void *buf[PCB_MAX_DEVICES] = {};
-    static size_t cap[PCB_MAX_DEVICES] = {};
-    const int dev = pcb_cur_device();
-    if (cap[dev] < bytes) {
-        void *fresh = nullptr;
-        if (cudaMalloc(&fresh, bytes) != cudaSuccess) { cudaGetLastError(); return nullptr; }
-        buf[dev] = fresh;
-        cap[dev] = bytes;
-    }
-    return static_cast<bf16 *>(buf[dev]);
-}
-
-}
-
-int pcb_k2r_weight_prepare(const pcb_conv *c, const K2rPlan &K, const float *w_master, void *w_fwd_extra, void *w_dg_extra, bool zero_padding,
-                           cudaStream_t st) {
-    PCB_CHECK(K.ok && w_fwd_extra && w_dg_extra, "k2r weight prepare: not a kernel-to-row layer / missing operand buffers");
-    float *wsub = reinterpret_cast<float *>(static_cast<bf16 *>(w_fwd_extra) + K.sub_fe);
-    k2r_weight_kernel<<<(K2R_N * K.cu + 255) / 256, 256, 0, st>>>(w_master, wsub, c->cout, c->cin, K.choff_u, K.cu);
-    PCB_LAUNCH_CHECK();
-    return pcb_tc_weight_prepare(&K.sub, wsub, w_fwd_extra, w_dg_extra, zero_padding, st);
-}
-
-int pcb_k2r_forward(const pcb_conv *c, const K2rPlan &K, const pcb_smallco_layout &L, const void *w_fwd, const void *w_fwd_extra, const float *bias,
-                    void *y, int y_cstride, const float *msum, void *workspace, cudaStream_t st) {
-    PCB_CHECK(K.ok && workspace, "k2r forward: not a kernel-to-row layer / no workspace");
+}
+
+int pcb_k2r_forward(const pcb_conv *c, const K2rPlan &K, const pcb_smallco_layout &L, const void *w_fwd, const float *bias, void *y, int y_cstride,
+                    const float *msum, cudaStream_t st) {
+    PCB_CHECK(K.ok && K.cu <= K2R_MAX_CU, "k2r forward: not a kernel-to-row layer");
     PCB_CHECK(y_cstride % 8 == 0 && y_cstride >= 8 && (reinterpret_cast<uintptr_t>(y) & 15) == 0, "small-cout forward: y must be 16-byte aligned with a channel stride that is a multiple of 8");
-    uint8_t *ws = static_cast<uint8_t *>(workspace);
-    bf16 *z = reinterpret_cast<bf16 *>(ws);
-    uint64_t *sub_ws = reinterpret_cast<uint64_t *>(ws + zbytes(c) + rup256(sizeof(float) * K2R_N * K.cu));
-    if (int rc = pcb_tc_forward_ws(&K.sub, w_fwd_extra, nullptr, z, K2R_N, nullptr, sub_ws, false, nullptr, nullptr, st)) return rc;
     K2rParams P;
     base(P, c, K);
-    P.z = z; P.w_fwd = static_cast<const bf16 *>(w_fwd); P.kf = L.kf; P.ktap = L.ktap; P.koff_s = L.koff[K.ps];
+    P.ups = (P.ks * 2 | 1) * 16;
+    P.w_fwd = static_cast<const bf16 *>(w_fwd); P.kf = L.kf; P.ktap = L.ktap; P.koff_u = L.koff[K.pu]; P.koff_s = L.koff[K.ps];
     P.bias = bias; P.msum = msum; P.y = static_cast<bf16 *>(y); P.y_cstride = y_cstride;
-    if (K.cs <= 3) k2r_combine_kernel<3><<<grid_for(c, 8), 256, 0, st>>>(P);
-    else k2r_combine_kernel<4><<<grid_for(c, 8), 256, 0, st>>>(P);
+    const size_t smem = std::max<size_t>(static_cast<size_t>(HROWS) * P.ups, static_cast<size_t>(HPIX) * ZS * 4) + static_cast<size_t>(K2R_N) * P.ups;
+    static Resident res[2][PCB_MAX_DEVICES] = {};
+    void (*kern)(const K2rParams) = K.cs <= 3 ? k2r_combine_kernel<3> : k2r_combine_kernel<4>;
+    kern<<<resident_grid(kern, smem, P.num_tiles, res[K.cs <= 3 ? 0 : 1]), THREADS, smem, st>>>(P);
     PCB_LAUNCH_CHECK();
     return 0;
 }
 
 int pcb_k2r_dgrad(const pcb_conv *c, const K2rPlan &K, const pcb_smallco_layout &L, const void *dc, int dc_cstride, const void *w_dgrad,
-                  const void *w_dg_extra, void *const *dx, const int *dx_cstride, cudaStream_t st) {
-    PCB_CHECK(K.ok, "k2r dgrad: not a kernel-to-row layer");
+                  void *const *dx, const int *dx_cstride, cudaStream_t st) {
+    PCB_CHECK(K.ok && K.cu <= K2R_MAX_CU, "k2r dgrad: not a kernel-to-row layer");
     PCB_CHECK(dc_cstride % 8 == 0 && dc_cstride >= 8, "small-cout dgrad: dc channel stride must be a multiple of 8");
     if (dx[K.pu]) {
-        bf16 *d = dgrad_scratch(zbytes(c));
-        PCB_CHECK(d != nullptr, "k2r dgrad: scratch allocation failed");
+        PCB_CHECK(dx_cstride[K.pu] % 8 == 0 && dx_cstride[K.pu] >= K.cu && (reinterpret_cast<uintptr_t>(dx[K.pu]) & 15) == 0,
+                  "k2r dgrad: dx must be 16-byte aligned with a channel stride that is a multiple of 8");
         K2rParams P;
         base(P, c, K);
-        P.dc = static_cast<const bf16 *>(dc); P.dc_cstride = dc_cstride; P.d = d;
-        k2r_dbuild_kernel<false, 3><<<grid_for(c, 8), 256, 0, st>>>(P);
+        P.dc = static_cast<const bf16 *>(dc); P.dc_cstride = dc_cstride;
+        P.w_dg = static_cast<const bf16 *>(w_dgrad); P.kd = L.kd; P.cout64 = L.cout64; P.koff_u = L.koff[K.pu];
+        P.du = static_cast<bf16 *>(dx[K.pu]); P.du_cstride = dx_cstride[K.pu];
+        static Resident res[PCB_MAX_DEVICES] = {};
+        k2r_dbuild_kernel<false, 3><<<resident_grid(k2r_dbuild_kernel<false, 3>, 0, P.num_tiles, res), THREADS, 0, st>>>(P);
         PCB_LAUNCH_CHECK();
-        void *dxs[1] = {dx[K.pu]};
-        const int cs[1] = {dx_cstride[K.pu]};
-        if (int rc = pcb_tc_dgrad(&K.sub, d, K2R_N, w_dg_extra, dxs, cs, st)) return rc;
     }
     if (dx[K.ps]) {
         void *dxl[2] = {nullptr, nullptr};
@@ -356,21 +601,21 @@
 }
 
 int pcb_k2r_wgrad(const pcb_conv *c, const K2rPlan &K, const void *dc, int dc_cstride, float *dw, void *workspace, bool zero_dw, cudaStream_t st) {
-    PCB_CHECK(K.ok && workspace, "k2r wgrad: not a kernel-to-row layer / no workspace");
-    PCB_CHECK(dc_cstride % 8 == 0 && dc_cstride >= 8, "small-cout wgrad: dc channel stride must be a multiple of 8");
+    PCB_CHECK(K.ok && K.cu <= K2R_MAX_CU && workspace, "k2r wgrad: not a kernel-to-row layer / no workspace");
+    PCB_CHECK(dc_cstride % 8 == 0 && dc_cstride >= 8 && (reinterpret_cast<uintptr_t>(dc) & 15) == 0,
+              "k2r wgrad: dc must be 16-byte aligned with a channel stride that is a multiple of 8");
     if (zero_dw) PCB_CUDA(cudaMemsetAsync(dw, 0, sizeof(float) * c->cout * K2R_TAPS * c->cin, st));
-    uint8_t *ws = static_cast<uint8_t *>(workspace);
-    bf16 *d = reinterpret_cast<bf16 *>(ws);
-    float *dwsub = reinterpret_cast<float *>(ws + zbytes(c));
-    void *sub_ws = ws + zbytes(c) + rup256(sizeof(float) * K2R_N * K.cu);
+    float *dwsub = static_cast<float *>(workspace);
+    PCB_CUDA(cudaMemsetAsync(dwsub, 0, sizeof(float) * K2R_K * K.cu, st));
     K2rParams P;
     base(P, c, K);
-    P.dc = static_cast<const bf16 *>(dc); P.dc_cstride = dc_cstride; P.d = d; P.dw = dw;
-    if (K.cs <= 3) k2r_dbuild_kernel<true, 3><<<grid_for(c, 3), 128, 0, st>>>(P);
-    else k2r_dbuild_kernel<true, 4><<<grid_for(c, 2), 128, 0, st>>>(P);
+    P.ups = ((K.cu / 8) | 1) * 16;
+    P.dc = static_cast<const bf16 *>(dc); P.dc_cstride = dc_cstride; P.dw = dw; P.dwsub = dwsub;
+    static Resident res[2][PCB_MAX_DEVICES] = {};
+    void (*kern)(const K2rParams) = K.cs <= 3 ? k2r_dbuild_kernel<true, 3> : k2r_dbuild_kernel<true, 4>;
+    kern<<<resident_grid(kern, 0, P.num_tiles, res[K.cs <= 3 ? 0 : 1]), THREADS, 0, st>>>(P);
     PCB_LAUNCH_CHECK();
-    if (int rc = pcb_tc_wgrad(&K.sub, d, K2R_N, dwsub, sub_ws, true, st)) return rc;
-    k2r_dw_scatter_kernel<<<(K2R_TAPS * K2R_CO * K.cu + 255) / 256, 256, 0, st>>>(dwsub, dw, c->cout, c->cin, K.choff_u, K.cu);
+    k2r_dw_scatter_kernel<<<(K2R_K * K.cu + 255) / 256, 256, 0, st>>>(dwsub, dw, c->cout, c->cin, K.choff_u, K.cu);
     PCB_LAUNCH_CHECK();
     return 0;
 }
diff --git a/text_segmentation_image_inpainting_b200/csrc/conv_tc.cu b/text_segmentation_image_inpainting_b200/csrc/conv_tc.cu
--- a/text_segmentation_image_inpainting_b200/csrc/conv_tc.cu
+++ b/text_segmentation_image_inpainting_b200/csrc/conv_tc.cu
@@ -2380,10 +2380,7 @@
     }
     PCB_LAUNCH_CHECK();
     if (T.fwd.route == ROUTE_STEM) return pcb_stem_weight_prepare(c, T.stem, w_master, wf + T.extra_fwd_off, zero_padding, st);
-    if (T.fwd.route == ROUTE_K2R) {
-        PCB_CHECK(w_dgrad != nullptr, "kernel-to-row weights need the dgrad operand buffer");
-        return pcb_k2r_weight_prepare(c, T.k2r, w_master, wf + T.extra_fwd_off, wd + T.extra_dg_off, zero_padding, st);
-    }
+    if (T.fwd.route == ROUTE_K2R) PCB_CHECK(w_dgrad != nullptr, "kernel-to-row layers need the dgrad operand buffer");
     if (T.sp.ok) {
         PCB_CHECK(w_dgrad != nullptr, "sub-pixel weights need the dgrad operand buffer");
         return sp_weight_prepare(c, T.sp, L, w_master, wd + T.sp_off, st);
@@ -2414,7 +2411,7 @@
         if (int rc = launch_tapmask(c, tapmask, st)) return rc;
     const bf16 *wf = static_cast<const bf16 *>(w_fwd);
     if (F.route == ROUTE_STEM) return pcb_stem_forward(c, T.stem, wf + T.extra_fwd_off, bias, y, y_cstride, msum, tapmask, bn_sums, ep, st);
-    if (F.route == ROUTE_K2R) return pcb_k2r_forward(c, T.k2r, smallco_layout(L), w_fwd, wf + T.extra_fwd_off, bias, y, y_cstride, msum, tapmask, st);
+    if (F.route == ROUTE_K2R) return pcb_k2r_forward(c, T.k2r, smallco_layout(L), w_fwd, bias, y, y_cstride, msum, st);
     if (F.route == ROUTE_SMALLCO) return pcb_smallco_forward(c, smallco_layout(L), w_fwd, bias, y, y_cstride, msum, st);
     TcParams P;
     base_params(P, c, L);
@@ -2454,7 +2451,7 @@
     PCB_CHECK(T.m_in < (1ll << 31), "problem too large");
     PCB_CHECK(dc_cstride % 8 == 0 && dc_cstride >= rup(c->cout, 8), "tensor-core dgrad: dc channel stride must be a multiple of 8");
     const bf16 *wd = static_cast<const bf16 *>(w_dgrad);
-    if (D.route == ROUTE_K2R) return pcb_k2r_dgrad(c, T.k2r, smallco_layout(L), dc, dc_cstride, w_dgrad, wd + T.extra_dg_off, dx, dx_cstride, st);
+    if (D.route == ROUTE_K2R) return pcb_k2r_dgrad(c, T.k2r, smallco_layout(L), dc, dc_cstride, w_dgrad, dx, dx_cstride, st);
     if (D.route == ROUTE_SMALLCO) return pcb_smallco_dgrad(c, smallco_layout(L), dc, dc_cstride, w_dgrad, dx, dx_cstride, st);
     const SpPlan &SPL = T.sp;
     void *dx_local[TC_MAX_PARTS] = {nullptr, nullptr};
diff --git a/text_segmentation_image_inpainting_b200/csrc/pcb_common.cuh b/text_segmentation_image_inpainting_b200/csrc/pcb_common.cuh
--- a/text_segmentation_image_inpainting_b200/csrc/pcb_common.cuh
+++ b/text_segmentation_image_inpainting_b200/csrc/pcb_common.cuh
@@ -159,12 +159,10 @@
     size_t workspace;
 };
 K2rPlan pcb_k2r_plan(const pcb_conv *c);
-int pcb_k2r_weight_prepare(const pcb_conv *c, const K2rPlan &K, const float *w_master, void *w_fwd_extra, void *w_dg_extra, bool zero_padding,
-                           cudaStream_t st);
-int pcb_k2r_forward(const pcb_conv *c, const K2rPlan &K, const pcb_smallco_layout &L, const void *w_fwd, const void *w_fwd_extra, const float *bias,
-                    void *y, int y_cstride, const float *msum, void *workspace, cudaStream_t st);
+int pcb_k2r_forward(const pcb_conv *c, const K2rPlan &K, const pcb_smallco_layout &L, const void *w_fwd, const float *bias, void *y, int y_cstride,
+                    const float *msum, cudaStream_t st);
 int pcb_k2r_dgrad(const pcb_conv *c, const K2rPlan &K, const pcb_smallco_layout &L, const void *dc, int dc_cstride, const void *w_dgrad,
-                  const void *w_dg_extra, void *const *dx, const int *dx_cstride, cudaStream_t st);
+                  void *const *dx, const int *dx_cstride, cudaStream_t st);
 int pcb_k2r_wgrad(const pcb_conv *c, const K2rPlan &K, const void *dc, int dc_cstride, float *dw, void *workspace, bool zero_dw, cudaStream_t st);
 struct StemPlan {
     bool ok;
```

New measurement: 1147 (median of 6 runs). 2.0% higher.
